# smdogroup/paropt

Measured on AMD Instinct MI355X. Metric: IP iterations/sec (KKT solve+line search), n=50M vars m=32, 1/2/4/8 GPUs, higher is better.
Workload: dtype f64

## Files before the change

paropt_amd/csrc/capi.cpp:

```cpp
#include <string.h>

#include "ip.hpp"
#include "problem.hpp"
#include "qn.hpp"

namespace po {
const char *last_error();
int ctx_create(int device, Ctx **out);
int ctx_destroy(Ctx *c);
int rccl_unique_id(void *id128);
int comm_init_rccl(Ctx *c, int rank, int size, const void *id128);
int comm_bench(Ctx *c, int count, int pure_sum, int reps, double out_us[3]);
int comm_allreduce_host(Ctx *c, double *values, int count, int op);
int rccl_version();
int comm_init_callback(Ctx *c, int rank, int size, po_allgather_fn fn, void *user);
}

using namespace po;

#define PO_CHECK_PTR(p)                         \
  do {                                          \
    if (!(p)) {                                 \
      po::set_error("null argument: %s", #p);   \
      return PO_ERR_ARG;                        \
    }                                           \
  } while (0)

static int same_layout(po_vec a, po_vec b) {
  if (a->ctx != b->ctx || a->n != b->n) {
    po::set_error("vector mismatch (different context or local size %lld vs %lld)", (long long)a->n,
                  (long long)b->n);
    return PO_ERR_ARG;
  }
  return PO_OK;
}

extern "C" {

const char *po_last_error(void) { return po::last_error(); }
const char *po_version(void) { return "paropt_amd 0.1 gfx950"; }

int po_ctx_create(int device, po_ctx *out) {
  PO_CHECK_PTR(out);
  Ctx *c = nullptr;
  int rc = ctx_create(device, &c);
  *out = static_cast<po_ctx>(c);
  return rc;
}
int po_ctx_destroy(po_ctx ctx) { return ctx_destroy(ctx); }
int po_ctx_synchronize(po_ctx ctx) {
  PO_CHECK_PTR(ctx);
  PO_HIP(hipStreamSynchronize(ctx->stream));
  return PO_OK;
}
int po_ctx_rank(po_ctx ctx, int *rank, int *size) {
  PO_CHECK_PTR(ctx);
  if (rank) *rank = ctx->rank;
  if (size) *size = ctx->size;
  return PO_OK;
}
void *po_ctx_stream(po_ctx ctx) { return ctx ? (void *)ctx->stream : nullptr; }
int po_ctx_counters(po_ctx ctx, int64_t *reductions, int64_t *launches) {
  PO_CHECK_PTR(ctx);
  if (reductions) *reductions = ctx->n_reductions;
  if (launches) *launches = ctx->n_launches;
  return PO_OK;
}
int po_ctx_sync_counters(po_ctx ctx, int64_t *flag_waits, int64_t *flag_timeouts, int64_t *allreduces,
                         int64_t *allgathers) {
  PO_CHECK_PTR(ctx);
  if (flag_waits) *flag_waits = ctx->n_flag_waits;
  if (flag_timeouts) *flag_timeouts = ctx->n_flag_timeouts;
  if (allreduces) *allreduces = ctx->n_allreduce;
  if (allgathers) *allgathers = ctx->n_allgather;
  return PO_OK;
}
int po_ctx_algorithmic_bytes(po_ctx ctx, double *total, double *user) {
  PO_CHECK_PTR(ctx);
  if (total) *total = ctx->alg_bytes;
  if (user) *user = ctx->alg_bytes_user;
  return PO_OK;
}
int po_debug_wgram_stamps(double *out8) { return po::wgram_debug_stamps(out8); }
int po_debug_set_switch(int id, int value) {
  po::dbg_switch_set(id, value);
  return PO_OK;
}

int po_ctx_set_reduction_batching(po_ctx ctx, int on) {
  PO_CHECK_PTR(ctx);
  PO_TRY(po::batch_flush(ctx));
  ctx->batch_enabled = on ? 1 : 0;
  return PO_OK;
}
int po_ctx_batched_reductions(po_ctx ctx, int64_t *batched) {
  PO_CHECK_PTR(ctx);
  if (batched) *batched = ctx->n_batched;
  return PO_OK;
}
int po_live_objects(int64_t *vectors, int64_t *bytes) {
  long v = 0;
  long long b = 0;
  po::live_objects(&v, &b);
  if (vectors) *vectors = v;
  if (bytes) *bytes = b;
  return PO_OK;
}
int po_device_count(int *count) {
  PO_CHECK_PTR(count);
  int n = 0;
  if (hipGetDeviceCount(&n) != hipSuccess) n = 0;
  *count = n;
  return PO_OK;
}
int po_options_visit_defaults(int which, po_option_visitor fn, void *user) {
  PO_CHECK_PTR(fn);
  po::Options o;
  po::Options base;
  if (which == 1) o.addTrustRegionDefaults();
  if (which == 2) o.addMMADefaults();
  if (which < 0 || which > 2) return PO_ERR_ARG;
  return o.visit(which == 0 ? nullptr : &base, fn, user);
}
int po_live_host_mirrors(int64_t *mirrors) {
  if (mirrors) *mirrors = po::live_mirrors();
  return PO_OK;
}
int po_ctx_time_mdot(po_ctx ctx, int nvecs) {
  PO_CHECK_PTR(ctx);
  ctx->time_mdot_nv = nvecs > 0 ? nvecs : 0;
  ctx->mdot_ms = 0.0;
  ctx->mdot_count = 0;
  return PO_OK;
}
int po_ctx_time_mdot_result(po_ctx ctx, double *ms_total, int64_t *launches) {
  PO_CHECK_PTR(ctx);
  if (ms_total) *ms_total = ctx->mdot_ms;
  if (launches) *launches = ctx->mdot_count;
  return PO_OK;
}
int po_ctx_time_wgram(po_ctx ctx, int on) {
  PO_CHECK_PTR(ctx);
  ctx->time_wgram = on ? 1 : 0;
  for (int i = 0; i < 2; i++) {
    ctx->wgram_ms[i] = 0.0;
    ctx->wgram_count[i] = 0;
    ctx->wgram_cols[i] = 0;
    ctx->wgram_bytes[i] = 0.0;
  }
  return PO_OK;
}
int po_ctx_time_wgram_result(po_ctx ctx, int which, double *ms_total, int64_t *launches, int *ncols,
                             double *alg_bytes_total) {
  PO_CHECK_PTR(ctx);
  if (which < 0 || which > 1) return PO_ERR_ARG;
  if (ms_total) *ms_total = ctx->wgram_ms[which];
  if (launches) *launches = ctx->wgram_count[which];
  if (ncols) *ncols = ctx->wgram_cols[which];
  if (alg_bytes_total) *alg_bytes_total = ctx->wgram_bytes[which];
  return PO_OK;
}
int po_ctx_comm_info(po_ctx ctx, int *kind, int64_t *allreduces, int64_t *allgathers) {
  PO_CHECK_PTR(ctx);
  if (kind) *kind = (int)ctx->comm_kind;
  if (allreduces) *allreduces = ctx->n_allreduce;
  if (allgathers) *allgathers = ctx->n_allgather;
// ... 1418 lines not shown
```

paropt_amd/csrc/context.cpp:

```cpp
#include <dlfcn.h>
#include <math.h>
#include <stdarg.h>
#include <execinfo.h>
#include <stdio.h>
#include <stdlib.h>
#include <string.h>
#include <time.h>

#include <algorithm>
#include <mutex>
#include <unordered_map>

#include "core.hpp"

namespace po {

static thread_local char g_err[1024] = "";
thread_local int g_last_code = 0;

void set_error(const char *fmt, ...) {
  va_list ap;
  va_start(ap, fmt);
  vsnprintf(g_err, sizeof(g_err), fmt, ap);
  va_end(ap);
  fprintf(stderr, "paropt_amd: %s\n", g_err);
}
const char *last_error() { return g_err; }

double host_now() {
  struct timespec t;
  clock_gettime(CLOCK_MONOTONIC, &t);
  return (double)t.tv_sec + 1e-9 * (double)t.tv_nsec;
}

struct SwitchDef {
  DbgSwitch id;
  const char *env;
  int dflt;
  bool presence;
};
static const SwitchDef kSwitches[] = {
    {SW_PERTURB_W, nullptr, 0, false},
    {SW_MPC_FUSE, "PAROPT_AMD_MPC_FUSE", 1, false},
    {SW_MPC_POLY, "PAROPT_AMD_MPC_POLY", 1, false},
    {SW_SPEC_DT, "PAROPT_AMD_SPEC_DT", 1, false},
    {SW_UNIFORM_BOUNDS, nullptr, 1, false},
    {SW_WGRAM_PRIO, "PAROPT_AMD_WGRAM_PRIO", 2, false},
    {SW_WGRAM_ABLATE, "PAROPT_AMD_WGRAM_ABLATE", 0, false},
    {SW_EXPLICIT_DOTS, "PAROPT_AMD_EXPLICIT_DOTS", 0, true},
    {SW_NO_RECOMPUTE, "PAROPT_AMD_NO_RECOMPUTE", 0, true},
    {SW_NO_RECOMPUTE_RHS, "PAROPT_AMD_NO_RECOMPUTE_RHS", 0, true},
    {SW_NO_FUSED_MERIT, "PAROPT_AMD_NO_FUSED_MERIT", 0, true},
    {SW_NO_LEAN_STEP, "PAROPT_AMD_NO_LEAN_STEP", 0, true},
    {SW_NO_RECOMPUTE_DT, "PAROPT_AMD_NO_RECOMPUTE_DT", 0, true},
    {SW_NO_FUSED_UPDATE, "PAROPT_AMD_NO_FUSED_UPDATE", 0, true},
    {SW_NO_CSR_GROUPS, "PAROPT_AMD_NO_CSR_GROUPS", 0, true},
    {SW_NO_FRONTS, "PAROPT_AMD_NO_FRONTS", 0, false},
    {SW_FORCE_RCCL, "PAROPT_AMD_FORCE_RCCL", 0, true},
    {SW_RCCL_ALLGATHER, "PAROPT_AMD_RCCL_ALLGATHER", 0, true},
    {SW_NO_DIRECT_RED, "PAROPT_AMD_NO_DIRECT_RED", 0, true},
    {SW_NO_FLAG_POLL, "PAROPT_AMD_NO_FLAG_POLL", 0, true},
    {SW_NO_BATCH, "PAROPT_AMD_NO_BATCH", 0, true},
    {SW_HOST_TRACE, "PAROPT_AMD_HOST_TRACE", 0, true},
    {SW_SYNC_TRACE, "PAROPT_AMD_SYNC_TRACE", 0, true},
    {SW_USER_TIMING, "PAROPT_AMD_USER_TIMING", 0, true},
    {SW_DUMP_LONG_SOLVES, "PAROPT_AMD_DUMP_LONG_SOLVES", -1, false},
};
static struct {
  int value = -1;
} g_dbg_switch[SW_COUNT];

int dbg_switch(DbgSwitch id) {
  if (g_dbg_switch[id].value >= 0) return g_dbg_switch[id].value;
  for (const SwitchDef &s : kSwitches) {
    if (s.id != id) continue;
    const char *e = s.env ? getenv(s.env) : nullptr;
    return e ? (s.presence ? 1 : atoi(e)) : s.dflt;
  }
  return 0;
}
void dbg_switch_set(int id, int value) {
  if (id >= 0 && id < SW_COUNT) g_dbg_switch[id].value = value;
}

int launch_reduce_final(Ctx *c, int nblocks, int nslots, int nsum, int nmin, int dst_off);
int launch_reduce_final_multi(Ctx *c, const Ctx::PendingRed *pend, int count);
int launch_red_publish(Ctx *c, const double *src, int count);
static int alloc_h_red(Ctx *c, size_t doubles) {
  if (c->h_red) (void)hipHostFree(c->h_red);
  c->h_red = nullptr;
  c->h_red_dev = nullptr;
  if (hipHostMalloc((void **)&c->h_red, sizeof(double) * doubles, hipHostMallocMapped | hipHostMallocCoherent) !=
      hipSuccess) {
    (void)hipGetLastError();
    c->h_red = nullptr;
    PO_HIP(hipHostMalloc((void **)&c->h_red, sizeof(double) * doubles, hipHostMallocDefault));
    c->h_red_coherent = 0;
  } else {
    c->h_red_coherent = 1;
  }
  if (dbg_switch(SW_NO_DIRECT_RED) ||
      hipHostGetDevicePointer((void **)&c->h_red_dev, c->h_red, 0) != hipSuccess) {
    (void)hipGetLastError();
    c->h_red_dev = nullptr;
  }
  if (c->h_flag && (!c->h_red_coherent || !c->h_red_dev)) {
    (void)hipHostFree(c->h_flag);
    c->h_flag = c->h_flag_dev = nullptr;
    if (c->d_ticket) (void)hipFree(c->d_ticket);
    c->d_ticket = nullptr;
  }
  if (c->h_red_dev && !c->h_flag && c->h_red_coherent && !dbg_switch(SW_NO_FLAG_POLL)) {
    if (hipHostMalloc((void **)&c->h_flag, 64, hipHostMallocMapped | hipHostMallocCoherent) == hipSuccess &&
        hipHostGetDevicePointer((void **)&c->h_flag_dev, c->h_flag, 0) == hipSuccess &&
        hipMalloc((void **)&c->d_ticket, sizeof(unsigned)) == hipSuccess &&
        hipMemset(c->d_ticket, 0, sizeof(unsigned)) == hipSuccess) {
      *c->h_flag = 0;
    } else {
      (void)hipGetLastError();
      if (c->h_flag) (void)hipHostFree(c->h_flag);
      if (c->d_ticket) (void)hipFree(c->d_ticket);
      c->h_flag = c->h_flag_dev = nullptr;
      c->d_ticket = nullptr;
    }
  }
  return PO_OK;
}


static int comm_self_test(Ctx *c);
static void free_overflow(Ctx *c, const double *keep);

struct Id128 {
  char b[PO_RCCL_ID_BYTES];
};
struct RcclApi {
  void *handle = nullptr;
  int (*GetUniqueId)(void *) = nullptr;
  int (*CommInitRank)(void **, int, Id128, int) = nullptr;
  int (*AllGather)(const void *, void *, size_t, int, void *, hipStream_t) = nullptr;
  int (*AllReduce)(const void *, void *, size_t, int, int, void *, hipStream_t) = nullptr;
  int (*CommDestroy)(void *) = nullptr;
  const char *(*GetErrorString)(int) = nullptr;
  int (*GetVersion)(int *) = nullptr;
  int version = 0;
};
static RcclApi g_rccl;

static int load_rccl() {
// ... 578 lines not shown
```

paropt_amd/csrc/core.hpp:

```cpp
#pragma once
#include <hip/hip_runtime.h>
#include <stdint.h>

#include <functional>
#include <string>
#include <vector>

#include "../../include/paropt_amd.h"

namespace po {

void set_error(const char *fmt, ...);
extern thread_local int g_last_code;

#define PO_HIP(expr)                                                                     \
  do {                                                                                   \
    hipError_t _e = (expr);                                                              \
    if (_e != hipSuccess) {                                                              \
      po::set_error("%s failed: %s (%s:%d)", #expr, hipGetErrorString(_e), __FILE__,     \
                    __LINE__);                                                           \
      return PO_ERR_HIP;                                                                 \
    }                                                                                    \
  } while (0)

#define PO_TRY(expr)            \
  do {                          \
    int _rc = (expr);           \
    if (_rc != PO_OK) return _rc; \
  } while (0)

constexpr int kBlock = 256;
constexpr int kMaxPanel = 96;
constexpr int kMaxRed = 8192;
constexpr int kWgramMaxVecs = 80;

enum CommKind { COMM_SELF = 0, COMM_RCCL = 1, COMM_CALLBACK = 2 };

struct Ctx {
  int device = 0;
  unsigned long long serial = 0;
  hipStream_t stream = nullptr;
  int num_cu = 256;
  int max_blocks = 2048;
  int rank = 0, size = 1;
  CommKind comm_kind = COMM_SELF;
  void *rccl_comm = nullptr;
  int rccl_allreduce = 1;
  long n_allreduce = 0, n_allgather = 0;
  po_allgather_fn cb_allgather = nullptr;
  void *cb_user = nullptr;
  double *d_partials = nullptr;
  double *partials_base = nullptr;
  size_t partials_cap = 0;
  size_t partials_cursor = 0;
  size_t partials_last = 0;
  double *d_red = nullptr;
  double *d_gather = nullptr;
  double *h_red = nullptr;
  double *h_red_dev = nullptr;
  unsigned long long *h_flag = nullptr, *h_flag_dev = nullptr;
  unsigned *d_ticket = nullptr;
  unsigned long long red_seq = 0, red_seq_seen = 0;
  int h_red_coherent = 0;
  long n_flag_waits = 0, n_flag_timeouts = 0;
  bool host_trace = false, host_gap_open = false;
  double host_t_sync = 0.0, host_gap_s = 0.0, host_launch_s = 0.0, host_wait_s = 0.0;
  long host_gap_n = 0, host_launch_n = 0, host_gap_n20 = 0, host_gap_long_n = 0;
  double host_gap_long_s = 0.0, host_t_launch_end = 0.0, host_inter_s = 0.0, host_inter_s30 = 0.0;
  long host_inter_n = 0, host_inter_n30 = 0;
  std::vector<double *> partials_overflow;
  hipEvent_t ev0 = nullptr, ev1 = nullptr;
  double *wide_scratch[2] = {nullptr, nullptr};
  int64_t wide_n = 0;
  hipEvent_t ev_mdot0 = nullptr, ev_mdot1 = nullptr;
  long n_reductions = 0;
  struct PendingRed {
    int off, nsum, nmin, nmax;
    double *host_out;
    const double *part;
    int nblocks;
  };
  int batch_enabled = 1;
  int batch_depth = 0;
  int batch_cursor = 0;
  std::vector<PendingRed> batch_pend;
  std::vector<std::function<void()>> batch_after;
  long n_batched = 0;
  long n_launches = 0;
  double alg_bytes = 0.0, alg_bytes_user = 0.0;
  int in_user = 0;
  int time_mdot_nv = 0;
  double mdot_ms = 0.0;
  long mdot_count = 0;
  bool mdot_timing_pending = false;
  int time_wgram = 0;
  double wgram_ms[2] = {0.0, 0.0};
  long wgram_count[2] = {0, 0};
  int wgram_cols[2] = {0, 0};
  double wgram_bytes[2] = {0.0, 0.0};
};

struct Vec {
  Ctx *ctx;
  int64_t n;
  double *d;
  int ref;
  double *h;
  int h_live = 0;
};

struct PtrTable {
  const double *p[kMaxPanel];
};
struct CoefTable {
  double a[kMaxPanel];
};
int reduce_finish(Ctx *c, int nblocks, int nsum, int nmin, int nmax, double *host_out, bool now = false,
                  double *local_out = nullptr);
bool red_direct(const Ctx *c);
int batch_flush(Ctx *c, const double *keep_partials = nullptr, size_t keep_len = 0);
void batch_abort(Ctx *c);
template <class F>
inline void after_reduce(Ctx *c, F &&f) {
  if (c->batch_depth > 0 && !c->batch_pend.empty()) {
    c->batch_after.emplace_back(std::forward<F>(f));
  } else {
    f();
  }
}
struct BatchScope {
  Ctx *c;
  bool open;
  explicit BatchScope(Ctx *c_, bool on = true) : c(c_), open(on && c_->batch_enabled) {
    if (open) c->batch_depth++;
  }
  void begin() {
    if (!open && c->batch_enabled) {
      open = true;
      c->batch_depth++;
    }
  }
  int end() {
    if (!open) return PO_OK;
    open = false;
    c->batch_depth--;
    return batch_flush(c);
  }
  int end_nested() {
    if (!open) return PO_OK;
    open = false;
    c->batch_depth--;
    return c->batch_depth > 0 ? PO_OK : batch_flush(c);
  }
  template <class F>
  int end_then(F &&post) {
    if (open) {
      open = false;
      c->batch_depth--;
      if (c->batch_depth > 0) {
        after_reduce(c, std::forward<F>(post));
        return PO_OK;
      }
      PO_TRY(batch_flush(c));
    }
    post();
    return PO_OK;
  }
  ~BatchScope() {
    if (open) {
      c->batch_depth--;
      batch_abort(c);
    }
  }
  BatchScope(const BatchScope &) = delete;
  BatchScope &operator=(const BatchScope &) = delete;
};
enum DbgSwitch {
  SW_PERTURB_W = 11, SW_MPC_FUSE = 14, SW_MPC_POLY = 15, SW_SPEC_DT = 16, SW_UNIFORM_BOUNDS = 17,
  SW_WGRAM_PRIO = 18, SW_WGRAM_ABLATE = 19, SW_EXPLICIT_DOTS = 20, SW_NO_RECOMPUTE = 21, SW_NO_RECOMPUTE_RHS = 22,
  SW_NO_FUSED_MERIT = 23, SW_NO_LEAN_STEP = 24, SW_NO_RECOMPUTE_DT = 25, SW_NO_FUSED_UPDATE = 26,
  SW_NO_CSR_GROUPS = 27, SW_NO_FRONTS = 28, SW_FORCE_RCCL = 29, SW_RCCL_ALLGATHER = 30, SW_NO_DIRECT_RED = 31,
  SW_NO_FLAG_POLL = 32, SW_NO_BATCH = 33, SW_HOST_TRACE = 34, SW_SYNC_TRACE = 35, SW_USER_TIMING = 36,
  SW_DUMP_LONG_SOLVES = 37, SW_COUNT = 38
};
int dbg_switch(DbgSwitch id);
void dbg_switch_set(int id, int value);
double host_now();
inline double host_trace_begin(Ctx *c);
inline void host_trace_end(Ctx *c, double t0);
int ensure_partials(Ctx *c, size_t doubles);
bool ctx_alive(const Ctx *c, unsigned long long serial);
inline double host_trace_begin(Ctx *c) {
  if (!c->host_trace) return 0.0;
  const double t = host_now();
  if (!c->host_gap_open && c->host_t_launch_end > 0.0) {
    const double g = t - c->host_t_launch_end;
    if (g < 500e-6) {
      c->host_inter_s += g;
      c->host_inter_n++;
      if (g > 30e-6) {
        c->host_inter_n30++;
        c->host_inter_s30 += g;
      }
    }
  }
  if (c->host_gap_open) {
    const double g = t - c->host_t_sync;
    if (g < 500e-6) {
      c->host_gap_s += g;
      c->host_gap_n++;
      if (g > 20e-6) c->host_gap_n20++;
    } else {
      c->host_gap_long_s += g;
      c->host_gap_long_n++;
    }
    c->host_gap_open = false;
  }
  return t;
}
inline void host_trace_end(Ctx *c, double t0) {
  if (!c->host_trace) return;
  c->host_t_launch_end = host_now();
  c->host_launch_s += c->host_t_launch_end - t0;
  c->host_launch_n++;
}
inline void count_bytes(Ctx *c, double streams, int64_t n) {
  const double b = 8.0 * streams * (double)n;
  c->alg_bytes += b;
  if (c->in_user) c->alg_bytes_user += b;
}
constexpr int kBpcPanel = 2;
constexpr int kBpcStream = 4;
int grid_for(Ctx *c, int64_t n);
int grid_for(Ctx *c, int64_t n, int bpc);

struct GroupCol {
  const double *w = nullptr;
  double scale = 0.0;
  unsigned period = 1, nw = 0;
  long long nwcon = 0;
};

struct GroupCols2 {
  GroupCol g[2];
  double ca[2] = {0.0, 0.0}, cb[2] = {0.0, 0.0};
  int count = 0;
};

int k_fill(Ctx *c, double *y, int64_t n, double alpha);
int k_fill_hash(Ctx *c, double *y, int64_t n, uint64_t seed, uint64_t aid, int64_t offset,
                double scale, double shift);
int k_copy(Ctx *c, double *y, const double *x, int64_t n);
int k_sign(Ctx *c, double *y, const double *x, int64_t n);
int k_scale(Ctx *c, double *y, int64_t n, double alpha);
int k_axpy(Ctx *c, double *y, double alpha, const double *x, int64_t n);
int k_panel_axpy(Ctx *c, double *y, double a, const double *x, double b, const double *alpha,
                 const double *const *V, int nv, int64_t n, const GroupCol *ybase = nullptr);
int k_panel_axpy2(Ctx *c, double *y1, double a1, const double *x1, const double *c1, double *y2, double a2,
                  const double *x2, const double *c2, const double *const *V, int nv, int64_t n);
int k_panel_lincomb(Ctx *c, double *const *dst, double a, const double *const *X, double b,
                    const double *const *Y, int nv, int64_t n);
enum Red1 { RED_DOT = 0, RED_SUMSQ = 1, RED_ASUM = 2, RED_AMAX = 3 };
int k_reduce1(Ctx *c, int kind, const double *x, const double *y, int64_t n, double *out);
int k_mdot(Ctx *c, const double *x, const double *const *V, int nv, int64_t n, double *out);
int k_minmax(Ctx *c, const double *x, int64_t n, double out[2]);
int k_stream_launch(Ctx *c, int kind, double *x, double *y, int64_t n);
int k_mdot_launch(Ctx *c, const double *x, const double *const *V, int nv, int64_t n, int *nblocks);
struct GramGroups {
  int64_t nwcon = 0, start = 0;
  int nw = 0, skip = 0;
  double alpha = 1.0;
  int ncols = 0;
  double *const *U = nullptr;
};
int k_wgram(Ctx *c, const double *d, const double *const *V, int nv, int64_t n, double *W,
            const double *const *S = nullptr, double *const *Zout = nullptr, int kpend = 0,
            double b0 = 0.0, int preweighted_last = 0, bool may_defer = false,
            const GramGroups *groups = nullptr, bool *groups_done = nullptr);
int wgram_debug_stamps(double out[8]);
int k_xgram(Ctx *c, const double *const *U, const double *const *Z, int m, int64_t w, double *out,
            bool may_defer = false);
int k_wgram_launch(Ctx *c, const double *d, const double *const *V, int nv, int64_t n,
                   int *nblocks, int *nslots, const double *const *S = nullptr,
                   double *const *Zout = nullptr, int kpend = 0, double b0 = 0.0,
                   int preweighted_last = 0, const GramGroups *groups = nullptr, bool *groups_done = nullptr);

struct Bounds {
  const double *x, *lb, *ub, *zl, *zu;
  double max_bound;
  int use_lower, use_upper;
  int lb_uni = 0, ub_uni = 0;
  double lb_c = 0.0, ub_c = 0.0;
};
inline int uniform_bound_streams(const Bounds &b) { return (b.lb_uni ? 1 : 0) + (b.ub_uni ? 1 : 0); }
struct ResidualSums {
  double comp_prod = 0, comp_count = 0, l1_rx = 0, l1_rzl = 0, l1_rzu = 0, l2_rx = 0, l2_rzl = 0, l2_rzu = 0;
  double max_rx = 0, max_rzl = 0, max_rzu = 0;
  double spec_max_rzl = 0, spec_max_rzu = 0;
  double *as_array() { return &comp_prod; }
};
static_assert(sizeof(ResidualSums) == 13 * sizeof(double), "k_kkt_res writes 13 slots");
struct KktResArgs {
  Bounds b;
  const double *g = nullptr;
  const double *const *A = nullptr;
  const double *z = nullptr;
  int nc = 0;
  double beta_mu = 0.0;
  int64_t n = 0;
  double *rx = nullptr;
  double *out = nullptr;
  double *yqn = nullptr;
  double beta_mu2 = -1.0;
  const GroupCol *gcol = nullptr;
  double gcoef = 0.0;
  struct Update {
    double *zl = nullptr;
    const double *pzl = nullptr;
    double *zu = nullptr;
    const double *pzu = nullptr;
    double a = 0.0, eps = 0.0;
    const double *va = nullptr;
    double az = 0.0;
    double *acz = nullptr;
    double az_acz = 0.0;
    const double *pxs = nullptr, *xold = nullptr;
    double beta_mu_step = 0.0;
    double *dinv_out = nullptr, *t_out = nullptr;
    double spec_diag = 0.0, spec_beta_mu = 0.0;
  } update;
};
int k_kkt_res(Ctx *c, const KktResArgs &o);
int k_kkt_res_update(Ctx *c, const KktResArgs &o);
int k_res_norms(Ctx *c, const Bounds &b, double beta_mu, int64_t n, double out[11]);
int k_dinv(Ctx *c, const Bounds &b, double diag, int64_t n, double *dinv,
           const double *hdiag = nullptr);
int k_d1s(Ctx *c, const Bounds &b, const double *bx, const double *dinv, double alpha, double beta_mu,
          int64_t n, double *t);
int k_solve2s(Ctx *c, const Bounds &b, const double *t, const double *dinv, const double *coef,
              const double *const *P, int nv, double alpha, double beta_mu, int full, double tau, int64_t n,
              double *px, double *pzl, double *pzu, double out[2]);
int k_d1(Ctx *c, const Bounds &b, const double *rx, const double *dinv, double beta_mu, int64_t n,
         double *t, const double *cl = nullptr, const double *cu = nullptr);
int k_dinv_d1(Ctx *c, const Bounds &b, double diag, const double *hdiag, const double *rx, double beta_mu,
              int64_t n, double *dinv, double *t, int raw = 0);
int k_corrector(Ctx *c, const Bounds &b, const double *px, const double *pzl, const double *pzu,
                int64_t n, double *cl, double *cu);
constexpr int kCorrDotsMax = 15;
int k_corr_d1_dots(Ctx *c, const Bounds &b, const double *px, const double *pzl, const double *pzu, const double *rx,
                   const double *dinv, double beta_mu, const double *const *V, int nv, int64_t n, double *t,
                   double *out);
struct CorrectorSums {
  double S10 = 0, S01 = 0, S11 = 0, ppos = 0, pneg = 0, gpx = 0, pxpx = 0, pos_log = 0, neg_log = 0;
  double max_x = 0, max_z = 0;
  double px_amax = 0;
  double *as_array() { return &S10; }
};
static_assert(sizeof(CorrectorSums) == 12 * sizeof(double), "k_solve2c writes 12 slots");
struct Solve2cArgs {
  Bounds b;
  const double *t = nullptr, *dinv = nullptr;
  const double *alpha = nullptr;
  const double *const *P = nullptr;
  int nv = 0;
  double beta_mu = 0.0, tau = 0.0;
  int64_t n = 0;
  double *px = nullptr, *pzl = nullptr, *pzu = nullptr;
  double *va = nullptr;
  int nca = 0;
  const double *g = nullptr;
  int want_logs = 0;
  double *out = nullptr;
};
int k_solve2c(Ctx *c, const Solve2cArgs &o);
struct Solve2Args {
  Bounds b;
  const double *t = nullptr, *dinv = nullptr;
// ... 131 lines not shown
```

paropt_amd/csrc/ip.cpp:

```cpp
#include "ip.hpp"

#include <math.h>
#include <stdio.h>
#include <stdlib.h>
#include <string.h>

#include <algorithm>
#include <chrono>

namespace po {

static const int LS_SUCCESS = 1, LS_FAILURE = 2, LS_MIN_STEP = 4, LS_MAX_ITERS = 8,
                 LS_NO_IMPROVEMENT = 16, LS_SHORT_STEP = 32;

InteriorPoint::InteriorPoint(Problem *p)
    : prob(p), ctx(p->ctx), n(p->nlocal), c(p->ncon), qn(nullptr), x(nullptr), zl(nullptr),
      zu(nullptr), lb(nullptr), ub(nullptr), g(nullptr), fobj(0.0), barrier_param(0.1),
      rho_penalty_search(0.0), niter(0), neval(0), ngeval(0),
      iter_cb(nullptr),
      iter_cb_user(nullptr), px(nullptr), pzl(nullptr), pzu(nullptr), Dinv(nullptr), rx(nullptr),
      tvec(nullptr), xt(nullptr), y_qn(nullptr), s_qn(nullptr), vA(nullptr), qn_created(false), qn_owned(true),
      comp_prod(0), comp_count(0), max_rx(0), max_rzl(0), max_rzu(0),
      corrector_active(false), norm_type(0), phase_t0(0) {
  qn_handle.qn = nullptr;
// ... 506 lines not shown
      mi = std::max(mi, fabs(r.z[i]));
      md = std::max(md, std::max(fabs(r.zs[i]), fabs(r.zt[i])));
    }
    if (use_lower) md = std::max(md, max_rzl);
    if (use_upper) md = std::max(md, max_rzu);
    if (has_w) {
      mi = std::max(mi, w_maxs[0]);
      md = std::max(md, std::max(std::max(w_maxs[1], w_maxs[2]), std::max(w_maxs[3], w_maxs[4])));
    }
  } else if (norm_type == 1) {
    mp = l1_rx;
    for (int i = 0; i < c; i++) {
      mp += fabs(r.s[i]);
      mp += fabs(r.t[i]);
      mi += fabs(r.z[i]);
      md += fabs(r.zs[i]);
      md += fabs(r.zt[i]);
    }
    if (use_lower) md += l1_rzl;
    if (use_upper) md += l1_rzu;
    if (has_w) {
      mi += w_sums[1];
      md += w_sums[3] + w_sums[4] + w_sums[5] + w_sums[6];
    }
  } else {
    double prime = 0.0, infeas = 0.0, dual = 0.0;
    for (int i = 0; i < c; i++) {
      prime += r.s[i] * r.s[i] + r.t[i] * r.t[i];
      infeas += r.z[i] * r.z[i];
      dual += r.zs[i] * r.zs[i] + r.zt[i] * r.zt[i];
    }
    mp = l2_rx + prime;
    mi = infeas;
    md = dual;
    if (use_lower) md += l2_rzl;
    if (use_upper) md += l2_rzu;
    if (has_w) {
      mi += w_sums[2];
      md += w_sums[3] * w_sums[3] + w_sums[4] * w_sums[4] + w_sums[5] * w_sums[5] +
            w_sums[6] * w_sums[6];
    }
    mp = sqrt(mp);
    mi = sqrt(mi);
    md = sqrt(md);
  }
  *max_prime = mp;
  *max_dual = md;
  *max_infeas = mi;
  *res_norm = std::max(mp, std::max(md, mi));
}

double InteriorPoint::compFromSums(double prod, double count, const Dense &v,
                                   double wprod) const {
  prod = prod / options.real("rel_bound_barrier");
  if (has_w) {
    prod += wprod;
    count += 2.0 * nw_global;
  }
  for (int i = 0; i < c; i++) {
    prod += v.s[i] * v.zs[i] + v.t[i] * v.zt[i];
    count += 2.0;
  }
  return count != 0.0 ? prod / count : 0.0;
}

int InteriorPoint::getComplementarity(double *comp) {
  double out[11];
  PO_TRY(k_res_norms(ctx, bounds(), 0.0, n, out));
  double wprod = 0.0;
  if (has_w) PO_TRY(wCompStep(0.0, 0.0, &wprod));
  *comp = compFromSums(out[0], out[1], vars, wprod);
  return PO_OK;
}

int InteriorPoint::formDinvAndRhs(double diag, bool use_hdiag, const double *rhs_mu, int kz, RhsFormed *formed) {
  const double *h = use_hdiag ? hdiag->d : nullptr;
  const double bmu = rhs_mu ? options.real("rel_bound_barrier") * (*rhs_mu) : 0.0;
  const bool want_t = rhs_mu && !has_w && c + kz > 0;
  const bool want_raw_d1 = has_w && rhs_mu && !corrector_active;
  const bool have_spec_dt = scratch_flags.spec_dt_valid;
  scratch_flags.spec_dt_valid = false;
  scratch_flags.t_is_plain_dinv_d1 = false;
  *formed = RHS_NONE;
  if (want_t) {
    const bool left_behind = have_spec_dt && !use_hdiag && spec_dt_diag == diag && spec_dt_bmu == bmu;
    if (!left_behind) PO_TRY(k_dinv_d1(ctx, bounds(), diag, h, rx->d, bmu, n, Dinv->d, tvec->d));
    scratch_flags.t_is_plain_dinv_d1 = !use_hdiag;
    t0_diag = diag;
    *formed = RHS_T;
  } else if (want_raw_d1) {
    PO_TRY(k_dinv_d1(ctx, bounds(), diag, h, rx->d, bmu, n, Dinv->d, d1v->d, 1));
    *formed = RHS_RAW_D1;
  } else {
    PO_TRY(k_dinv(ctx, bounds(), diag, n, Dinv->d, h));
  }
  return PO_OK;
}

int InteriorPoint::gramPass(const GramPlan &plan, bool *groups_done) {
  const int m = (int)plan.V.size(), mt = m + (plan.with_t ? 1 : 0), k = plan.kform;
  const bool with_t = plan.with_t;
  std::vector<const double *> V(plan.V);
  if (with_t) V.push_back(tvec->d);
  Wt_buf.assign((size_t)mt * mt, 0.0);
  PO_TRY(k_wgram(ctx, Dinv->d, V.data(), mt, n, Wt_buf.data(), k > 0 ? plan.S.data() : nullptr,
                 k > 0 ? plan.Zout.data() : nullptr, k, plan.b0, with_t ? 1 : 0, plan.may_defer, plan.groups,
                 groups_done));
  t0dots.assign(with_t ? m : 0, 0.0);
  after_reduce(ctx, [this, m, mt, k, with_t] {
    auto at = [&](int i) { return k == 0 ? i : (i < c ? k + i : i - c); };
    for (int j = 0; j < m; j++)
      for (int i = 0; i < m; i++) kkt.W[i + (size_t)m * j] = Wt_buf[at(i) + (size_t)mt * at(j)];
    for (int i = 0; with_t && i < m; i++) t0dots[i] = Wt_buf[at(i) + (size_t)mt * m];
  });
  return PO_OK;
}

int InteriorPoint::setUpKKTSystem(bool use_qn, bool diag_only, const double *rhs_mu) {
  if (qn) PO_TRY(refreshQuasiNewton());
  step_flags.ptpx_valid = false;
  scratch_flags.t0_valid = false;
  const bool use_hdiag = options.integer("use_diag_hessian") && hdiag;
  const double b0 = (!use_hdiag && qn && (use_qn || diag_only)) ? qn->diag() : 0.0;
  const bool with_z = use_qn && !diag_only;
  RhsFormed rhs = RHS_NONE;
  PO_TRY(formDinvAndRhs(b0 + options.real("qn_sigma"), use_hdiag, rhs_mu, (qn && with_z) ? qn->size() : 0, &rhs));
  const bool fuse_t = rhs == RHS_T, raw_d1_w = rhs == RHS_RAW_D1;
  GramPlan plan;
  std::vector<const double *> Yp, Sp;
  std::vector<double *> Zo;
  double b0z = 0.0;
  const bool fuse_z = qn && with_z && !has_w && qn->pendingZ(&Yp, &Sp, &Zo, &b0z) && !Yp.empty() && Yp.size() <= 12 &&
                      c + (int)Yp.size() + (fuse_t ? 1 : 0) <= kWgramMaxVecs;
  int k = 0;
  std::vector<const double *> P;
  if (fuse_z) {
    plan.kform = k = (int)Yp.size();
    plan.V = Yp;
    for (Vec *a : Ac) plan.V.push_back(a->d);
    plan.S = Sp;
    plan.Zout = Zo;
    plan.b0 = b0z;
  } else {
    plan.V = P = panel(with_z, &k);
  }
  const int m = c + k;
  kkt.k = k;
  bool fuse_tw = false;
  BatchScope wbatch(ctx, has_w && prob->reductionsBatchable());
  if (has_w) {
    PO_TRY(prob->sparseFactorFromSlacks(x, Dinv, wv(), Cw));
    fuse_tw = rhs_mu && m > 0 && m + 1 <= kWgramMaxVecs && !corrector_active;
    if (fuse_tw) {
      PO_TRY(computeResidualW(*rhs_mu, true, true));
      if (!raw_d1_w)
        PO_TRY(k_d1(ctx, bounds(), rx->d, nullptr, options.real("rel_bound_barrier") * (*rhs_mu), n, d1v->d));
      PO_TRY(applyK0(d1v->d, wd2->d, tvec, wyw));
    }
  }
  GramGroups gram_groups;
  std::vector<double *> Ugs;
  if (has_w && m > 0 && prob->sparseGramGroups(x, &gram_groups)) {
    PO_TRY(panelImageVectors(m, Ugs));
    gram_groups.ncols = m;
    gram_groups.U = Ugs.data();
    plan.groups = &gram_groups;
  }
  plan.with_t = (fuse_t || fuse_tw) && m > 0 && m + 1 <= kWgramMaxVecs;
  plan.may_defer = wbatch.open;
  bool panel_done = false;
  kkt.W.assign((size_t)m * m, 0.0);
  t0dots.clear();
  if (m > 0) PO_TRY(gramPass(plan, &panel_done));
  if (fuse_z) qn->pendingZDone();
  if (plan.with_t) {
    scratch_flags.t0_valid = true;
    t0_mu = *rhs_mu;
  }
  if (has_w) PO_TRY(sparseGramCorrection(P, m, fuse_tw ? d1v : tvec, wbatch.open, panel_done));
  PO_TRY(wbatch.end());
  if (m > 1 && debug_keep_schur && dbg_switch(SW_PERTURB_W) != 0) {
    kkt.W[1] *= 1.0 + 1e-9;
    kkt.W[m] = kkt.W[1];
  }
  const double *d0 = nullptr, *M = nullptr;
  if (k > 0) {
    double b0_;
    qn->getCompactMat(&b0_, &d0, &M, nullptr);
  }
  kkt.factor(vars, d0, M, debug_keep_schur ? &Gmat0 : nullptr, debug_keep_schur ? &Ce0 : nullptr);
  if (k == 0) Ce0.clear();
  return PO_OK;
}

int InteriorPoint::solveKKT(const Dense &b, double mu, bool use_qn, bool refine_pass, double tau,
                            Dense &out, bool fuse_residual) {
  const double beta_mu = options.real("rel_bound_barrier") * mu;
  const int k = (qn && use_qn) ? qn->size() : 0;
  PO_TRY(kkt.checkWidth(k));
  const int m = c + k;
  std::vector<const double *> P;
  bool have_panel = false;
  auto need_panel = [&]() {
    if (!have_panel) {
      int k2 = 0;
      P = panel(use_qn, &k2);
      have_panel = true;
    }
  };
  const bool corr = corrector_active && !refine_pass;
  const bool corr_fused = corr && corrector_fused && m >= 1 && m <= kCorrDotsMax;
  const double *cl = (corr && !corr_fused) ? s_qn->d : nullptr;
  const double *cu = (corr && !corr_fused) ? y_qn->d : nullptr;
  if (corr && corrector_fused && !corr_fused) {
    set_error("internal: fused corrector solve with a panel of %d columns", m);
    return PO_ERR_ARG;
  }
  const bool have_t0 = !refine_pass && scratch_flags.t0_valid && t0_mu == mu && !corr && (int)t0dots.size() == m;
  std::vector<double> dots(m > 0 ? m : 1, 0.0);
  if (corr_fused) {
    need_panel();
    PO_TRY(k_corr_d1_dots(ctx, bounds(), px->d, pzl->d, pzu->d, rx->d, Dinv->d, beta_mu, P.data(), m, n, tvec->d,
                          dots.data()));
  } else {
    if (!refine_pass && !have_t0) PO_TRY(k_d1(ctx, bounds(), rx->d, Dinv->d, beta_mu, n, tvec->d, cl, cu));
    if (have_t0) {
      for (int i = 0; i < m; i++) dots[i] = t0dots[i];
    } else if (refine_pass && step_flags.tdots_valid && (int)tdots.size() == m) {
      dots = tdots;
    } else if (m > 0) {
      need_panel();
      PO_TRY(k_mdot(ctx, tvec->d, P.data(), m, n, dots.data()));
    }
  }
  if (!refine_pass) scratch_flags.first_t_recomputable = have_t0 && scratch_flags.t_is_plain_dinv_d1;
  if (!refine_pass) scratch_flags.t0_valid = false;
  const bool deferred = refine_pass && step_flags.step_deferred;
  const Bordered::Sol sol = solveBordered(b, dots.data(), refine_pass);
  const bool seq_lin = options.integer("sequential_linear_method");
  const int kq = (qn && !seq_lin) ? qn->size() : 0;
  const bool fuse = fuse_residual && !refine_pass && forms.analytic_panel_dots && kq == k &&
                    !options.integer("use_diag_hessian") && !inexact_newton_step && m <= kMaxPanel;
  step_flags.vA_valid = true;
  std::vector<double> coef(m > 0 ? m : 1, 0.0);
  double diag = options.real("qn_sigma");
  if (fuse) PO_TRY(residualCoefs(qn && !seq_lin ? RES_QN : RES_SIGMA, sol.coef.data(), ptpx.data() + c, k, coef, &diag));
  need_panel();
  const SolvePass sp{P, sol.coef, m, beta_mu, tau};
  if (fuse && m > 0 && !corr) {
    PO_TRY(fusedFirstPass(sp, coef, diag));
  } else if (deferred) {
    PO_TRY(recomputingRefinementPass(sp, corr));
  } else if (corr_fused) {
    PO_TRY(correctorSolve(sp));
  } else {
    PO_TRY(storedStepSolve(sp, refine_pass, fuse ? coef.data() : nullptr, diag, cl, cu));
  }
  step_flags.residual_fused = fuse;
  kkt.backSubstitute(1.0, b, vars, sol, true, out);
  return PO_OK;
}

Bordered::Sol InteriorPoint::solveBordered(const Dense &b, const double *dots, bool refine_pass) {
  stepWillChange();
  Bordered::Sol sol;
  kkt.solve(1.0, b, vars, dots, &sol);
  kkt.panelDots(dots, sol, refine_pass, &ptpx);
  step_flags.ptpx_valid = true;
  return sol;
}

int InteriorPoint::fusedFirstPass(const SolvePass &sp, const std::vector<double> &coef, double diag) {
  const int m = sp.m;
  std::vector<double> out(m + 2, 0.0);
  const bool defer = forms.recompute_first_step;
  double *tp_out = !defer ? tvec->d : (forms.recompute_rhs ? nullptr : xt->d);
  const bool redo_dt1 = forms.recompute_dt && defer && forms.recompute_rhs && scratch_flags.first_t_recomputable;
  PO_TRY(k_solve2_dots(ctx, {.b = bounds(), .t = redo_dt1 ? nullptr : tvec->d, .dinv = Dinv->d,
                             .alpha = sp.alpha.data(), .coef2 = coef.data(), .P = sp.P.data(), .nv = m,
                             .beta_mu = sp.beta_mu, .tau = sp.tau, .rx = rx->d, .diag = diag, .n = n, .px = px->d,
                             .pzl = pzl->d, .pzu = pzu->d, .tout = tp_out, .va = vA->d, .nca = c, .out = out.data(),
                             .store_step = defer ? 0 : 1, .dinv_diag = t0_diag}));
  tdots.assign(out.begin(), out.begin() + m);
  step_flags.tdots_valid = true;
  step_mins[0] = out[m];
  step_mins[1] = out[m + 1];
  step_flags.step_deferred = defer;
  if (defer) {
    alpha_first = sp.alpha;
    coef_first = coef;
    diag_first = diag;
  }
  return PO_OK;
}

int InteriorPoint::recomputingRefinementPass(const SolvePass &sp, bool corr) {
  const bool take_merit = forms.fuse_merit && forms.recompute_rhs && !corr;
  const bool lean = forms.lean_step && lean_step_allowed && take_merit && iterate_flags.iterate_logs_valid;
  const bool redo_dt = forms.recompute_dt && forms.recompute_rhs && scratch_flags.first_t_recomputable;
  if (lean) {
    step_flags.pz_stored = false;
    step_beta_mu = sp.beta_mu;
  }
  PO_TRY(k_solve2r(ctx, {.b = bounds(), .t1 = redo_dt ? nullptr : tvec->d,
                         .t2 = forms.recompute_rhs ? nullptr : xt->d, .dinv = Dinv->d, .a1 = alpha_first.data(),
                         .a2 = sp.alpha.data(), .P = sp.P.data(), .nv = sp.m, .beta_mu = sp.beta_mu, .tau = sp.tau,
                         .n = n, .px = px->d, .pzl = lean ? nullptr : pzl->d, .pzu = lean ? nullptr : pzu->d,
                         .va = vA->d, .nca = c, .out = step_mins, .ar = coef_first.data(), .rx = rx->d,
                         .diag = diag_first, .g = take_merit ? g->d : nullptr,
                         .merit_out = take_merit ? fused_merit.as_array() : nullptr, .dinv_diag = t0_diag}));
  if (take_merit) {
    after_reduce(ctx, [this] {
      step_mins[0] = fused_merit.max_x;
      step_mins[1] = fused_merit.max_z;
      step_flags.fused_merit_valid = true;
    });
  }
  return PO_OK;
}

int InteriorPoint::correctorSolve(const SolvePass &sp) {
  const bool want_logs = !iterate_flags.iterate_logs_valid;
  PO_TRY(k_solve2c(ctx, {.b = bounds(), .t = tvec->d, .dinv = Dinv->d, .alpha = sp.alpha.data(), .P = sp.P.data(),
                         .nv = sp.m, .beta_mu = sp.beta_mu, .tau = sp.tau, .n = n, .px = px->d, .pzl = pzl->d,
                         .pzu = pzu->d, .va = vA->d, .nca = c, .g = g->d, .want_logs = want_logs ? 1 : 0,
                         .out = corr_out.as_array()}));
  after_reduce(ctx, [this, want_logs] {
    const CorrectorSums &o = corr_out;
    fused_merit = {.S10 = o.S10, .S01 = o.S01, .S11 = o.S11, .ppos = o.ppos, .pneg = o.pneg, .gpx = o.gpx,
                   .pxpx = o.pxpx, .max_x = o.max_x, .max_z = o.max_z, .px_amax = o.px_amax};
    step_mins[0] = o.max_x;
    step_mins[1] = o.max_z;
    if (want_logs) {
      iterate_logs[0] = o.pos_log;
      iterate_logs[1] = o.neg_log;
      iterate_flags.iterate_logs_valid = true;
    }
    step_flags.fused_merit_valid = true;
  });
  return PO_OK;
}

int InteriorPoint::storedStepSolve(const SolvePass &sp, bool refine_pass, const double *coef2, double diag,
                                   const double *cl, const double *cu) {
  return k_solve2(ctx, {.b = bounds(), .t = tvec->d, .dinv = Dinv->d, .alpha = sp.alpha.data(), .P = sp.P.data(),
                        .nv = sp.m, .beta_mu = sp.beta_mu, .refine = refine_pass ? 1 : 0, .tau = sp.tau, .n = n,
                        .px = px->d, .pzl = pzl->d, .pzu = pzu->d, .out = step_mins, .coef2 = coef2, .rx = rx->d,
                        .diag = diag, .tout = tvec->d, .va = vA->d, .nca = c, .cl = cl, .cu = cu});
}

int InteriorPoint::computeKKTStepWithRefinement(double mu, bool use_qn, double tau) {
  const int nref = options.integer("iterative_refinement_steps");
  const double beta_mu = options.real("rel_bound_barrier") * mu;
  const bool with_qn = qn && !options.integer("sequential_linear_method");
  const int mq = c + (with_qn ? qn->size() : 0);
  const bool diag_hess = options.integer("use_diag_hessian") && (!has_w || hdiag);
  const ResTerm term = (!has_w && inexact_newton_step) ? RES_HVEC
                       : diag_hess                     ? RES_HDIAG
                       : with_qn                       ? RES_QN
                                                       : RES_SIGMA;
  if (has_w && !(scratch_flags.t0_valid && t0_mu == mu)) PO_TRY(computeResidualW(mu));
  denseResidual(mu, res);
  PO_TRY(has_w ? solveKKTW(res, mu, use_qn, false, tau, step, nref > 0)
               : solveKKT(res, mu, use_qn, false, tau, step, nref > 0));
  for (int it = 0; it < nref; it++) {
    LazyPanel Pq{this, with_qn};
    if (has_w) Pq.get();
    std::vector<double> dots;
    PO_TRY(stepPanelDots(Pq, dots));
    std::vector<double> coef(mq + 2, 0.0);
    double diag = 0.0;
    PO_TRY(residualCoefs(term, step.z.data(), dots.data() + c, mq - c, coef, &diag));
    int mres = mq;
    if (term == RES_HVEC || term == RES_HDIAG) {
      Pq.get().push_back(xt->d);
      mres++;
    }
    if (!(it == 0 && step_flags.residual_fused)) {
      if (has_w) {
        if (prob->setSparseJacobianTranspose(1.0, x, wstepv[0], tvec) != 0) return PO_ERR_USER;
        Pq.get().push_back(tvec->d);
        coef[mres++] = 1.0;
      }
      PO_TRY(k_res_step(ctx, bounds(), rx->d, px->d, pzl->d, pzu->d, has_w ? nullptr : Dinv->d, coef.data(),
                        Pq.get().data(), mres, diag, beta_mu, n, has_w ? d1v->d : tvec->d));
    }
    if (has_w) {
      PO_TRY(computeResidualW(mu, false));
      if (prob->addSparseJacobian(-1.0, x, px, wresv[0]) != 0) return PO_ERR_USER;
      PO_TRY(k_w_res_step(ctx, wv(), wp(), wr(), nw, wd2->d));
      scratch_flags.wd2_ready = true;
    }
    Dense r2;
    r2.resize(c);
    denseResidual(mu, r2);
    denseResStep(vars, step, dots.data(), r2);
    PO_TRY(has_w ? solveKKTW(r2, mu, use_qn, true, tau, refine) : solveKKT(r2, mu, use_qn, true, tau, refine));
    for (int i = 0; i < c; i++) {
      step.z[i] += refine.z[i];
      step.s[i] += refine.s[i];
      step.t[i] += refine.t[i];
      step.zs[i] += refine.zs[i];
      step.zt[i] += refine.zt[i];
    }
  }
  sx = sz = 1.0;
  return PO_OK;
}

int InteriorPoint::checkKKTStep(int iteration, double mu) {
  const double beta_mu = options.real("rel_bound_barrier") * mu;
  if (!step_flags.pz_stored) {
    PO_TRY(k_form_pz(ctx, bounds(), px->d, step_beta_mu, n, pzl->d, pzu->d));
    step_flags.pz_stored = true;
  }
  const bool seq_lin = options.integer("sequential_linear_method");
  int kq = 0;
  std::vector<const double *> Pq = panel(qn && !seq_lin, &kq);
  const int mq = c + kq;
  std::vector<double> dots(mq > 0 ? mq : 1, 0.0), coef(mq > 0 ? mq : 1, 0.0);
  if (mq > 0) PO_TRY(k_mdot(ctx, px->d, Pq.data(), mq, n, dots.data()));
  double diag = 0.0;
  const bool with_qn = qn && !seq_lin && !options.integer("use_diag_hessian");
  PO_TRY(residualCoefs(with_qn ? RES_QN : RES_SIGMA, step.z.data(), dots.data() + c, kq, coef, &diag));
  if (has_w) {
    if (prob->setSparseJacobianTranspose(1.0, x, wstepv[0], xt) != 0) return PO_ERR_USER;
    Pq.push_back(xt->d);
    coef.push_back(1.0);
  }
  double mx[3];
  PO_TRY(computeResidual(mu, true));
  PO_TRY(k_step_check(ctx, bounds(), rx->d, px->d, pzl->d, pzu->d, coef.data(), Pq.data(), (int)Pq.size(), diag,
                      beta_mu, n, mx));
  Dense r;
  r.resize(c);
  denseResidual(mu, r);
  denseResStep(vars, step, dots.data(), r);
  double mz = 0.0, ms = 0.0, mt = 0.0, mzs = 0.0, mzt = 0.0;
  for (int i = 0; i < c; i++) {
    mz = std::max(mz, fabs(r.z[i]));
    ms = std::max(ms, fabs(r.s[i]));
    mt = std::max(mt, fabs(r.t[i]));
    mzs = std::max(mzs, fabs(r.zs[i]));
    mzt = std::max(mzt, fabs(r.zt[i]));
  }
  if (ctx->rank == 0) {
    char line[640];
    snprintf(line, sizeof(line),
             "\nResidual step check for iteration %d:\n"
             "max |stationarity (x block)|:             %10.4e\n"
             "max |dense constraints (z block)|:        %10.4e\n"
             "max |slack duals (s block)|:              %10.4e\n"
             "max |slack duals (t block)|:              %10.4e\n"
             "max |slack complementarity (zs block)|:   %10.4e\n"
             "max |slack complementarity (zt block)|:   %10.4e\n"
             "max |lower-bound complementarity (zl)|:   %10.4e\n"
             "max |upper-bound complementarity (zu)|:   %10.4e\n",
             iteration, mx[0], mz, ms, mt, mzs, mzt, mx[1], mx[2]);
    history += line;
  }
  return PO_OK;
}

int InteriorPoint::checkGradients(double dh, std::string *report) {
  scratchLent();
  return prob->checkGradients(dh, x, options.integer("use_hvec_product"), xt, tvec, report);
// ... 1342 lines not shown
```

paropt_amd/csrc/ip.hpp:

```cpp
#pragma once
#include <stdlib.h>
#include <map>
#include <string>
#include <vector>

#include "bordered.hpp"
#include "problem.hpp"
#include "qn.hpp"

namespace po {

class Options {
 public:
  enum Type { STR = 1, BOOL = 2, INT = 3, FLOAT = 4, ENUM = 5 };
  struct Entry {
    Type type;
    std::string s;
    int i = 0, ilo = 0, ihi = 0;
    double f = 0, flo = 0, fhi = 0;
    std::vector<std::string> choices;
  };
  Options();
  void addTrustRegionDefaults();
  void addMMADefaults();
  int set(const char *name, const char *value);
  int set(const char *name, int value);
  int set(const char *name, double value);
  const char *str(const char *name) const;
  int integer(const char *name) const;
  double real(const char *name) const;
  bool has(const char *name) const { return e.count(name) > 0; }
  int visit(const Options *skip, po_option_visitor fn, void *user) const;
  void adoptExtras(const Options &src, const Options &base);

 private:
  std::map<std::string, Entry> e;
};

class InteriorPoint {
 public:
  InteriorPoint(Problem *prob);
  ~InteriorPoint();
  int allocate();
  const std::vector<int> &gPivots() const { return kkt.gpiv; }
  Vec *lowerBounds() { return lb; }
  Vec *upperBounds() { return ub; }
  void clearUniformBounds() { bounds_uni[0] = bounds_uni[1] = 0; }
  int checkFlag() const { return check_flag; }
  int clampCounts(double out[8]);
  int checkKKTStep(int iteration, double mu);

  Options options;
  int optimize(const char *checkpoint);
  void getOptimizedPoint(Vec **x, const double **z, Vec **zl, Vec **zu);
  void getOptimizedSlacks(const double **s, const double **t, const double **zs, const double **zt);
  void getOptimizedSparse(Vec *v[5]);
  void getIterationCounters(int *niter_, int *neval_, int *ngeval_);
  double getBarrierParameter() const { return barrier_param; }
  int getComplementarity(double *comp);
  void setPenaltyGamma(double gamma);
  void setPenaltyGammaArray(const double *gamma);
  int resetDesignAndBounds();
  void resetQuasiNewtonHessian();
  int setQuasiNewton(CompactQuasiNewton *qn_);
  int resetProblemInstance(Problem *p);
  int writeSolutionFile(const char *filename);
  int readSolutionFile(const char *filename);
  int debugKKTStep(double mu);
  int debugSetState(const double *z, const double *s, const double *t, const double *zs, const double *zt, double mu);
  int debugKKT(double mu, int mode, double tau);
  std::vector<double> Gmat0, Ce0;
  bool debug_keep_schur = false;
  double debug_norms[4] = {0, 0, 0, 0};
  const std::vector<double> &gramMatrix() const { return kkt.W; }
  const std::vector<int> &cPivots() const { return kkt.cpiv; }
  const double *stepMins() const { return step_mins; }
  Vec *dinvVec() { return Dinv; }
  Vec *rxVec() { return rx; }
  void flushHistory();
  int checkGradients(double dh, std::string *report);
  int checkMeritFuncGradient(Vec *xpt, double dh, double out[2]);
  int setHvecFiniteDifference(int mode, int central, double rel_step);
  void getHvecFiniteDifferenceCount(int *products, int *evaluations) const;
  double hvecFiniteDifferenceStep() const { return hvec_fd_h; }
  int evalHvec(const double *z, Vec *zw, Vec *p, Vec *hvec);

  Problem *prob;
  Ctx *ctx;
  int64_t n;
  int c;
  CompactQuasiNewton *qn;
  po_qn_s qn_handle;

  Vec *x, *zl, *zu, *lb, *ub, *g;
  std::vector<Vec *> Ac;
  Dense vars, res, step, refine;
  double fobj, barrier_param, rho_penalty_search;
  std::vector<double> cvals;
  int niter, neval, ngeval, nhvec;

  po_ip_iteration_fn iter_cb;
  void *iter_cb_user;
  std::string history;
  std::vector<std::string> phase_names;
  std::vector<double> phase_seconds;
  std::string phase_names_joined;
  bool user_timing = dbg_switch(SW_USER_TIMING) != 0;

  Vec *px, *pzl, *pzu;

  int64_t nw;
  bool has_w;
  double nw_global;
  Vec *wvar[5], *wresv[5], *wstepv[5];

 private:
  Vec *Dinv, *rx, *tvec, *xt, *y_qn, *s_qn;
  Vec *vA;
  std::vector<double> gamma_s, gamma_t;
  int use_lower, use_upper;
  bool qn_created;
  bool qn_owned;

  Bordered kkt;
  std::vector<double> Wt_buf, W2_buf;
  Bordered::Sol solveBordered(const Dense &b, const double *dots, bool refine_pass);
  struct SolvePass {
    const std::vector<const double *> &P;
    const std::vector<double> &alpha;
    int m;
    double beta_mu, tau;
  };

  struct StepFlags {
    bool ptpx_valid = false;
    bool tdots_valid = false;
    bool merit_cache_valid = false;
    bool fused_merit_valid = false;
    bool px_amax_valid = false;
    bool w_comp_valid = false;
    bool w_merit_cache_valid = false;
    bool vA_valid = false;
    bool residual_fused = false;
    bool pz_stored = true;
    bool step_deferred = false;
    bool px_first_only = false;
  } step_flags;
  std::vector<double> ptpx;
  std::vector<double> tdots;
  MeritSums merit_cache;
  FusedMeritSums fused_merit;
  CorrectorSums corr_out;
  double px_amax_w = 0.0;
  double w_step_out[5] = {0, 0, 0, 0, 0}, w_comp_poly[3] = {0, 0, 0}, w_merit_cache[10] = {0};
  bool lean_step_allowed = false;
  double step_beta_mu = 0.0;
  std::vector<double> alpha_first, coef_first;
  double diag_first = 0.0;
  double step_mins[2];
  double sx = 1.0, sz = 1.0;

  struct ScratchFlags {
    bool spec_dt_valid = false;
    bool t0_valid = false;
    bool t_is_plain_dinv_d1 = false;
    bool first_t_recomputable = false;
    bool wd2_ready = false;
    bool panel_valid = false;
  } scratch_flags;
  bool spec_dt_want = false;
  double spec_dt_diag = 0.0, spec_dt_bmu = 0.0, spec_dt_mu = 0.0;
  double t0_mu = 0.0;
  std::vector<double> t0dots;
  double t0_diag = 0.0;

  struct IterateFlags {
    bool ac_valid = false;
    bool acz_valid = false;
    bool cwx_valid = false;
    bool trial_cw_valid = false;
    bool iterate_logs_valid = false;
    bool trial_logs_valid = false;
    bool residual_cached = false;
    bool spec_valid = false;
    bool s_qn_from_trial = false;
  } iterate_flags;
  static const int kAczRefresh = 16;
  Vec *acz = nullptr;
  int acz_age = 0;
  double trial_logs[2] = {0, 0}, iterate_logs[2] = {0, 0};
  bool spec_enabled = false;
  double spec_mu = 0.0, spec_max[2] = {0.0, 0.0};
  double s_qn_a = 0.0;

  void stepWillChange() { step_flags = {}; }
  void scratchLent() { scratch_flags = {}; }
  void iterateReplaced() { iterate_flags = {}; }
  void stateReplaced() {
    stepWillChange();
    scratchLent();
    iterateReplaced();
  }

  ResidualSums res_out;
  double wres_out[12] = {0};
  double comp_prod, comp_count, max_rx, max_rzl, max_rzu;
  double l1_rx = 0, l1_rzl = 0, l1_rzu = 0, l2_rx = 0, l2_rzl = 0, l2_rzu = 0;
  bool corrector_active;
  bool corrector_fused = false;
  int norm_type;

  Vec *hdiag;
  std::vector<Vec *> gmresW;
  bool inexact_newton_step;
  int gatherCounts(int64_t mine, std::vector<int64_t> *all);
  int solutionFileOffsets(int64_t *nvars_total, int64_t *var_off, int64_t *nw_total, int64_t *w_off);
  int ensureHdiag();
  int solveKKTAlpha(const double *bx, double alpha, const Dense &b, double mu, bool use_qn, bool full,
                    double tau, Dense &out);
  int evalObjBarrierDeriv(const Dense &p, double *pmerit);
  int solveKKTAlphaW(const double *bx, double alpha, const Dense &b, double mu, bool use_qn, bool full,
                     double tau, Dense &out);
  Vec *wscalev[5];
  double w_merit_last[10];
  int computeKKTGMRESStep(double rtol, double atol, bool use_qn, double tau, int *gmres_iters);

  int hvec_mode = PO_HVEC_EXACT, hvec_central = 0;
  double hvec_rel = 0.0;
  bool hvec_fd_active = false;
  int hvec_fd_products = 0, hvec_fd_evals = 0;
  double hvec_fd_h = 0.0;
  Vec *hvec_xp = nullptr;
  std::vector<Vec *> hvec_work[2];
  Vec *hvec_csr_data = nullptr, *hvec_csr_cw = nullptr;
  int64_t hvec_csr_nnz = 0;
  int hvecProduct(const double *z, Vec *zw, Vec *p, Vec *hvec);
  int hvecFiniteDifference(const double *z, Vec *zw, Vec *p, Vec *hvec);
  int hvecScratch(int sides, int nc);
  int hvecEvalAt(double a, Vec *p, int side, bool with_jac);

  Vec *gsw, *gtw, *Cw, *wd2, *wyw, *wtmp, *wtmp2;
  Vec *cwx = nullptr;
  int sparseConAtIterate(const double **cw);
  Vec *d1v;
  std::vector<Vec *> Uw;
  GramForm panel_form = {false, false};
  std::vector<Vec *> Yw;
  std::vector<const double *> correctionPanel(int m) const;
  double w_sums[7], w_maxs[5];
  double nextMonotoneMu() const;
  WVars wv() const;
  WVars wr() const;
  WVars wp() const;
  int allocateW();
  int applyK0(const double *bx, const double *bw, Vec *yx, Vec *yw);
  int computeResidualW(double mu, bool norms = true, bool with_d2 = false);
  int sparseGramCorrection(const std::vector<const double *> &P, int m, Vec *work = nullptr, bool may_defer = false,
                           bool panel_done = false);
  int panelImageVectors(int m, std::vector<double *> &U);
  int solveKKTW(const Dense &b, double mu, bool use_qn, bool refine_pass, double tau, Dense &out,
                bool fuse_residual = false);
  int fusedFirstPassW(const SolvePass &sp, int k, double mins_x[2], double mins_w[2]);
  int correctionPanelSolve(const SolvePass &sp, bool refine_pass, bool first_px_only, const double *cl,
                           const double *cu, double mins_x[2], double mins_w[2]);
  int blockSolveFallback(const SolvePass &sp, bool refine_pass, const double *cl, const double *cu, double mins_x[2],
                         double mins_w[2]);
  int initLeastSquaresMultipliersW();
  int wCompStep(double ax, double az, double *prod);

  Bounds bounds() const;
  std::vector<const double *> panel(bool use_qn, int *k) const;
  struct LazyPanel {
    const InteriorPoint *ip;
    bool use_qn;
    bool asked = false;
    std::vector<const double *> P;
    std::vector<const double *> &get();
  };
  int stepPanelDots(LazyPanel &P, std::vector<double> &dots);
  std::vector<double> compactInverse(const double *ztp, int kq) const;
  enum ResTerm { RES_SIGMA, RES_QN, RES_HVEC, RES_HDIAG };
  int residualCoefs(ResTerm term, const double *z, const double *ztpx, int kq, std::vector<double> &coef,
                    double *diag);

  int createQuasiNewton();
  int refreshQuasiNewton();
  int initAndCheckDesignAndBounds();
  int initLeastSquaresMultipliers();
  int initAffineStepMultipliers();
  void denseResidual(double mu, Dense &r) const;
  struct MultUpdate {
    double a = 0.0, az = 0.0, eps = 0.0;
    bool acz_follow = false;
  };
  int computeResidual(double mu, bool vectors, Vec *yqn_complete = nullptr, const MultUpdate *upd = nullptr);
  void resNorms(const Dense &r, double *max_prime, double *max_dual, double *max_infeas,
                double *res_norm) const;
  double compFromSums(double prod, double count, const Dense &v, double wprod = 0.0) const;
  int setUpKKTSystem(bool use_qn, bool diag_only = false, const double *rhs_mu = nullptr);
  enum RhsFormed { RHS_NONE, RHS_T, RHS_RAW_D1 };
  int formDinvAndRhs(double diag, bool use_hdiag, const double *rhs_mu, int kz, RhsFormed *formed);
  struct GramPlan {
    std::vector<const double *> V;
    int kform = 0;
    std::vector<const double *> S;
    std::vector<double *> Zout;
    double b0 = 0.0;
    bool with_t = false;
    const GramGroups *groups = nullptr;
    bool may_defer = false;
  };
  int gramPass(const GramPlan &plan, bool *groups_done);
  int solveKKT(const Dense &b, double mu, bool use_qn, bool refine_pass, double tau, Dense &out,
               bool fuse_residual = false);
  int fusedFirstPass(const SolvePass &sp, const std::vector<double> &coef, double diag);
  int recomputingRefinementPass(const SolvePass &sp, bool corr);
  int correctorSolve(const SolvePass &sp);
  int storedStepSolve(const SolvePass &sp, bool refine_pass, const double *coef2, double diag, const double *cl,
                      const double *cu);
  int computeKKTStepWithRefinement(double mu, bool use_qn, double tau);
  int mehrotraStep(bool use_qn, double comp, bool corrector, double min_frac, double abs_res_tol, double *tau_out);
  int scaleKKTStep(double tau, double comp, double *alpha_x, double *alpha_z, int *ceq,
                   bool inexact = false);
  int evalMeritInitDeriv(double max_x, double *merit, double *pmerit);
  double evalMeritFromSums(double fk, const double *ck, const double *sk, const double *tk,
                           double pos, double neg, const double *wsums = nullptr) const;
  int lineSearch(double alpha_min, double *alpha, double m0, double dm0, int *fail);
  int computeStepAndUpdate(double alpha, int eval_obj_con, int perform_qn_update, int *update_type);
  void phaseBegin();
  void phaseEnd(const char *name);
  double phase_t0;
  static const int kUserRing = 16;
  hipEvent_t user_ev[2 * kUserRing];
  int user_pending = 0;
  bool user_events_ready = false;
  double user_seconds = 0.0;
  void userBegin();
  void userEnd();
  void userHarvest();
  struct Forms {
    bool analytic_panel_dots;
    bool fuse_merit;
    bool lean_step;
    bool recompute_dt;
    bool recompute_first_step;
    bool recompute_rhs;
    bool fuse_mult_update;
  };
  static Forms readForms();
  const Forms forms = readForms();
  int check_flag = 0;
  int bounds_uni[2] = {0, 0};
  double bounds_val[2] = {0.0, 0.0};
};

}

struct po_ip_s {
  po::InteriorPoint *ip;
};
```

paropt_amd/csrc/ip_gmres.cpp:

```cpp
#include <math.h>

#include <algorithm>

#include "ip.hpp"

namespace po {

int InteriorPoint::ensureHdiag() {
  if (hdiag) return PO_OK;
  hdiag = vec_new(ctx, n);
  return hdiag ? PO_OK : PO_ERR_HIP;
}

int InteriorPoint::solveKKTAlpha(const double *bx, double alpha, const Dense &b, double mu, bool use_qn,
                                 bool full, double tau, Dense &out) {
  const double beta_mu = options.real("rel_bound_barrier") * mu;
  int k = 0;
  std::vector<const double *> P = panel(use_qn, &k);
  PO_TRY(kkt.checkWidth(k));
  const int m = c + k;
  PO_TRY(k_d1s(ctx, bounds(), bx, Dinv->d, alpha, beta_mu, n, tvec->d));
  std::vector<double> dots(m > 0 ? m : 1, 0.0);
  if (m > 0) PO_TRY(k_mdot(ctx, tvec->d, P.data(), m, n, dots.data()));
  Bordered::Sol sol;
  kkt.solve(alpha, b, vars, dots.data(), &sol);
  const std::vector<double> &coef = sol.coef;
  stepWillChange();
  kkt.panelDots(dots.data(), sol, false, &ptpx);
  step_flags.ptpx_valid = true;
  PO_TRY(k_solve2s(ctx, bounds(), tvec->d, Dinv->d, coef.data(), P.data(), m, alpha, beta_mu, full ? 1 : 0, tau,
                   n, px->d, pzl->d, pzu->d, step_mins));
  kkt.backSubstitute(alpha, b, vars, sol, full, out);
  return PO_OK;
}

int InteriorPoint::solveKKTAlphaW(const double *bx, double alpha, const Dense &b, double mu, bool use_qn,
                                  bool full, double tau, Dense &out) {
  const double beta_mu = options.real("rel_bound_barrier") * mu;
  int k = 0;
  std::vector<const double *> P = panel(use_qn, &k);
  PO_TRY(kkt.checkWidth(k));
  const int m = c + k;
  WVars ws{wscalev[0]->d, wscalev[1]->d, wscalev[2]->d, wscalev[3]->d, wscalev[4]->d};
  PO_TRY(k_d1s(ctx, bounds(), bx, nullptr, alpha, beta_mu, n, d1v->d));
  PO_TRY(k_w_scale5(ctx, ws, wr(), alpha, nw));
  PO_TRY(k_w_d2(ctx, wv(), ws, nw, wd2->d));
  PO_TRY(applyK0(d1v->d, wd2->d, tvec, wyw));
  std::vector<double> dots(m > 0 ? m : 1, 0.0);
  if (m > 0) PO_TRY(k_mdot(ctx, tvec->d, P.data(), m, n, dots.data()));
  Bordered::Sol sol;
  kkt.solve(alpha, b, vars, dots.data(), &sol);
  const std::vector<double> &coef = sol.coef;
  stepWillChange();
  kkt.panelDots(dots.data(), sol, false, &ptpx);
  step_flags.ptpx_valid = true;
  double mins_w[2] = {1.0, 1.0};
  if (!full && k > 0) {
    if (c > 0) {
      PO_TRY(k_panel_axpy(ctx, xt->d, 1.0, d1v->d, 0.0, sol.yz.data(), P.data(), c, n));
      PO_TRY(applyK0(xt->d, wd2->d, tvec, wyw));
    }
    PO_TRY(k_w_step(ctx, wv(), ws, wyw->d, 0, tau, wp(), nw, mins_w));
    PO_TRY(k_panel_axpy(ctx, d1v->d, 0.0, nullptr, 1.0, coef.data(), P.data(), m, n));
    PO_TRY(applyK0(d1v->d, wd2->d, tvec, wtmp2));
  } else {
    if (m > 0) PO_TRY(k_panel_axpy(ctx, d1v->d, 0.0, nullptr, 1.0, coef.data(), P.data(), m, n));
    PO_TRY(applyK0(d1v->d, wd2->d, tvec, wyw));
    PO_TRY(k_w_step(ctx, wv(), ws, wyw->d, 0, tau, wp(), nw, mins_w));
  }
  double mins_x[2] = {1.0, 1.0};
  PO_TRY(k_solve2s(ctx, bounds(), tvec->d, Dinv->d, coef.data(), P.data(), 0, alpha, beta_mu, full ? 1 : 0, tau,
                   n, px->d, pzl->d, pzu->d, mins_x));
  step_mins[0] = std::min(mins_x[0], mins_w[0]);
  step_mins[1] = std::min(mins_x[1], mins_w[1]);
  kkt.backSubstitute(alpha, b, vars, sol, full, out);
  return PO_OK;
}

int InteriorPoint::evalObjBarrierDeriv(const Dense &p, double *pmerit_) {
  const double beta = options.real("rel_bound_barrier");
  double out[6];
  PO_TRY(k_merit0(ctx, bounds(), px->d, 1.0, g->d, n, out));
  double ppos = out[2] * beta, pneg = out[3] * beta;
  if (has_w) {
    const double *cw = nullptr;
    PO_TRY(sparseConAtIterate(&cw));
    PO_TRY(k_fill(ctx, wtmp2->d, nw, 0.0));
    if (prob->addSparseJacobian(1.0, x, px, wtmp2) != 0) return PO_ERR_USER;
    PO_TRY(k_w_merit(ctx, wv(), wp(), 1.0, gsw->d, gtw->d, cw, wtmp2->d, nw, w_merit_last));
    ppos += w_merit_last[2];
    pneg += w_merit_last[3];
  }
  for (int i = 0; i < c; i++) {
    if (p.s[i] > 0.0) ppos += p.s[i] / vars.s[i]; else pneg += p.s[i] / vars.s[i];
    if (p.t[i] > 0.0) ppos += p.t[i] / vars.t[i]; else pneg += p.t[i] / vars.t[i];
  }
  double pmerit = out[4] - barrier_param * (ppos + pneg);
  for (int i = 0; i < c; i++) pmerit += gamma_s[i] * p.s[i] + gamma_t[i] * p.t[i];
  if (has_w) pmerit += w_merit_last[6] + w_merit_last[7];
  *pmerit_ = pmerit;
  return PO_OK;
}

// ... 172 lines not shown
```

paropt_amd/csrc/kernels.hip:

```cpp
#include "core.hpp"

#include <math.h>
#include <stdlib.h>
#include <string.h>

namespace po {

#define PO_PAIR_LOOP(q, n)                                                                 \
  const int64_t _npairs = ((n) + 1) >> 1;                                                  \
  for (int64_t q = (int64_t)blockIdx.x * blockDim.x + threadIdx.x; q < _npairs;            \
       q += (int64_t)gridDim.x * blockDim.x)

typedef double f64x2l __attribute__((ext_vector_type(2)));
__device__ __forceinline__ double2 ld2(const double *__restrict__ p, int64_t q, int64_t n) {
#ifndef PO_LD2_PLAIN
  const f64x2l v = __builtin_nontemporal_load(reinterpret_cast<const f64x2l *>(p + 2 * q));
  return make_double2(v.x, v.y);
#else
  return *reinterpret_cast<const double2 *>(p + 2 * q);
#endif
}
#ifndef PO_ST2_PLAIN
#define PO_ST2_NT 1
#endif
typedef double f64x2s __attribute__((ext_vector_type(2)));
__device__ __forceinline__ void st2(double *__restrict__ p, int64_t q, int64_t n, double2 v) {
  if (2 * q + 1 >= n) v.y = 0.0;
#ifdef PO_ST2_NT
  __builtin_nontemporal_store((f64x2s){v.x, v.y}, reinterpret_cast<f64x2s *>(p + 2 * q));
#else
  *reinterpret_cast<double2 *>(p + 2 * q) = v;
#endif
}

typedef double f64x4 __attribute__((ext_vector_type(4)));
typedef double f64x2 __attribute__((ext_vector_type(2)));

__device__ __forceinline__ f64x2 ld_stream(const double *p) {
  return __builtin_nontemporal_load(reinterpret_cast<const f64x2 *>(p));
}

enum { OP_SUM = 0, OP_MIN = 1, OP_MAX = 2 };

template <int OP>
__device__ __forceinline__ double combine(double a, double b) {
  if (OP == OP_SUM) return a + b;
  if (OP == OP_MIN) return fmin(a, b);
  return fmax(a, b);
}

template <int OP>
__device__ __forceinline__ double wave_reduce(double v) {
#pragma unroll
  for (int o = 32; o > 0; o >>= 1) v = combine<OP>(v, __shfl_xor(v, o, 64));
  return v;
}

template <int N, int OP>
__device__ __forceinline__ void block_reduce_store(double (&a)[N], double *__restrict__ partials,
                                                   int slot0, double *sm) {
  const int lane = threadIdx.x & 63, wave = threadIdx.x >> 6;
#pragma unroll
  for (int j = 0; j < N; j++) {
    double v = wave_reduce<OP>(a[j]);
    if (lane == 0) sm[wave * N + j] = v;
  }
  __syncthreads();
  if (threadIdx.x < N) {
    const int j = threadIdx.x;
    double v = combine<OP>(combine<OP>(sm[j], sm[N + j]), combine<OP>(sm[2 * N + j], sm[3 * N + j]));
    partials[(size_t)(slot0 + j) * gridDim.x + blockIdx.x] = v;
  }
  __syncthreads();
}

__device__ __forceinline__ void red_raise_flag(volatile unsigned long long *flag, unsigned long long seq,
                                               unsigned *ticket) {
  if (!flag) return;
  __threadfence_system();
  __syncthreads();
  if (threadIdx.x == 0) {
    const unsigned t = atomicAdd(ticket, 1u);
    if (t == gridDim.x - 1) {
// ... 623 lines not shown
  __shared__ double sm[4 * NVB];
  double acc[NVB];
  const double *vp[NVB];
#pragma unroll
  for (int j = 0; j < NVB; j++) {
    acc[j] = 0.0;
    vp[j] = V.p[j0 + j];
  }
  PO_PAIR_LOOP(q, n) {
    const f64x2 xv = *reinterpret_cast<const f64x2 *>(x + 2 * q);
#pragma unroll
    for (int j = 0; j < NVB; j++) {
      const f64x2 w = ld_stream(vp[j] + 2 * q);
      acc[j] = fma(xv.x, w.x, fma(xv.y, w.y, acc[j]));
    }
  }
  block_reduce_store<NVB, OP_SUM>(acc, partials, j0, sm);
}

#define PO_MDOT_CASE(NVB)                                                          \
  case NVB:                                                                        \
    PO_LAUNCH(mdot_kernel<NVB>, grid, x, pt, j0, n, c->d_partials);                \
    break;

int k_mdot_launch(Ctx *c, const double *x, const double *const *V, int nv, int64_t n, int *nblocks) {
  count_bytes(c, nv + 1, n);
  if (nv > kMaxPanel) {
    set_error("mdot of %d vectors exceeds kMaxPanel=%d", nv, kMaxPanel);
    return PO_ERR_ARG;
  }
  const int grid = grid_for(c, n, 5);
  PO_TRY(ensure_partials(c, (size_t)grid * (nv + 32)));
  PtrTable pt;
  CoefTable ct;
  fill_tables(nullptr, V, nv, &ct, &pt);
  int j0 = 0;
  while (j0 < nv) {
    const int rem = nv - j0;
    const int w = rem >= 32 ? 32 : (rem >= 24 ? 24 : (rem >= 16 ? 16 : rem));
    switch (w) {
      PO_MDOT_CASE(1) PO_MDOT_CASE(2) PO_MDOT_CASE(3) PO_MDOT_CASE(4) PO_MDOT_CASE(5)
      PO_MDOT_CASE(6) PO_MDOT_CASE(7) PO_MDOT_CASE(8) PO_MDOT_CASE(9) PO_MDOT_CASE(10)
      PO_MDOT_CASE(11) PO_MDOT_CASE(12) PO_MDOT_CASE(13) PO_MDOT_CASE(14) PO_MDOT_CASE(15)
      PO_MDOT_CASE(16) PO_MDOT_CASE(24) PO_MDOT_CASE(32)
    }
    j0 += w;
  }
  *nblocks = grid;
  return PO_OK;
}

int k_mdot(Ctx *c, const double *x, const double *const *V, int nv, int64_t n, double *out) {
  if (nv <= 0) return PO_OK;
  if (nv > kMaxPanel) {
    for (int j0 = 0; j0 < nv; j0 += kMaxPanel)
      PO_TRY(k_mdot(c, x, V + j0, nv - j0 > kMaxPanel ? kMaxPanel : nv - j0, n, out + j0));
    return PO_OK;
  }
  int grid = 0;
  const bool timed = c->time_mdot_nv == nv;
  if (timed && c->mdot_timing_pending) PO_TRY(batch_flush(c));
  if (timed) PO_HIP(hipEventRecord(c->ev_mdot0, c->stream));
  PO_TRY(k_mdot_launch(c, x, V, nv, n, &grid));
  if (timed) PO_HIP(hipEventRecord(c->ev_mdot1, c->stream));
  const bool defer = timed && c->batch_depth > 0;
  PO_TRY(reduce_finish(c, grid, nv, 0, 0, out, timed && !defer));
  if (timed) {
    auto harvest = [c] {
      float ms = 0.0f;
      if (hipEventSynchronize(c->ev_mdot1) == hipSuccess &&
          hipEventElapsedTime(&ms, c->ev_mdot0, c->ev_mdot1) == hipSuccess) {
        c->mdot_ms += ms;
        c->mdot_count++;
      }
      c->mdot_timing_pending = false;
    };
    if (defer) c->mdot_timing_pending = true;
    after_reduce(c, harvest);
  }
  return PO_OK;
}


struct BE {
  bool L, U;
  double xl, xu, zl, zu;
};
__device__ __forceinline__ BE bound_elem(double x, double lb, double ub, double zl, double zu,
                                         double maxb, int use_lower, int use_upper) {
  BE e;
  e.L = use_lower && (lb > -maxb);
  e.U = use_upper && (ub < maxb);
  e.xl = e.L ? (x - lb) : 1.0;
  e.xu = e.U ? (ub - x) : 1.0;
  e.zl = zl;
  e.zu = zu;
  return e;
}
#define PO_MAKE_BOUNDS(b, q, n)                                                          \
  const bool _has2 = (2 * q + 1 < n);                                                    \
  const BE e0 = bound_elem(_x.x, _lb.x, _ub.x, _zl.x, _zu.x, (b).max_bound, (b).use_lower, \
                           (b).use_upper);                                               \
  BE e1 = bound_elem(_x.y, _lb.y, _ub.y, _zl.y, _zu.y, (b).max_bound, (b).use_lower,     \
                     (b).use_upper);                                                     \
  if (!_has2) {                                                                          \
    e1.L = false;                                                                        \
    e1.U = false;                                                                        \
    e1.xl = 1.0;                                                                         \
    e1.xu = 1.0;                                                                         \
  }
__device__ __forceinline__ double2 ld2_bound(const double *__restrict__ p, int uni, double v, int64_t q, int64_t n) {
  return uni ? make_double2(v, v) : ld2(p, q, n);
}
#define PO_LD2_LB(b, q, n) ld2_bound((b).lb, (b).lb_uni, (b).lb_c, q, n)
#define PO_LD2_UB(b, q, n) ld2_bound((b).ub, (b).ub_uni, (b).ub_c, q, n)
#define PO_LOAD_BOUNDS(b, q, n)                                                         \
  const double2 _x = ld2((b).x, q, n), _lb = PO_LD2_LB(b, q, n), _ub = PO_LD2_UB(b, q, n), \
                _zl = ld2((b).zl, q, n), _zu = ld2((b).zu, q, n);                        \
  PO_MAKE_BOUNDS(b, q, n)

__device__ __forceinline__ void res_bound_acc(const BE &e, double beta_mu, double *sums, double *maxs,
                                              int il1, int il2, int imax) {
  if (e.L) {
    sums[0] += e.zl * e.xl;
    sums[1] += 1.0;
    const double r = fabs(-(e.xl * e.zl - beta_mu));
    sums[il1] += r;
    sums[il2] += r * r;
    maxs[imax] = fmax(maxs[imax], r);
  }
  if (e.U) {
    sums[0] += e.zu * e.xu;
    sums[1] += 1.0;
    const double r = fabs(-(e.xu * e.zu - beta_mu));
    sums[il1 + 1] += r;
    sums[il2 + 1] += r * r;
    maxs[imax + 1] = fmax(maxs[imax + 1], r);
  }
}
__device__ __forceinline__ void res_bound_max2(const BE &e, double beta_mu2, double *m2) {
  if (e.L) m2[0] = fmax(m2[0], fabs(-(e.xl * e.zl - beta_mu2)));
  if (e.U) m2[1] = fmax(m2[1], fabs(-(e.xu * e.zu - beta_mu2)));
}
__global__ void __launch_bounds__(kBlock)
    kkt_res_kernel(Bounds b, const double *__restrict__ g, PtrTable A, CoefTable z, int nc,
                   double beta_mu, int64_t n, double *__restrict__ rx, double *__restrict__ yqn,
                   double beta_mu2, GroupCol gcol, double gcoef, double *__restrict__ partials) {
  __shared__ double sm[4 * 8];
  double sums[8] = {0.0, 0.0, 0.0, 0.0, 0.0, 0.0, 0.0, 0.0};
  double maxs[5] = {0.0, 0.0, 0.0, 0.0, 0.0};
  PO_PAIR_LOOP(q, n) {
    PO_LOAD_BOUNDS(b, q, n);
    const double2 gv = ld2(g, q, n);
    double2 yv = make_double2(0.0, 0.0);
    if (yqn) yv = ld2(yqn, q, n);
    double2 r;
    r.x = (b.use_lower ? _zl.x : 0.0);
    r.y = (b.use_lower ? _zl.y : 0.0);
    if (b.use_upper) {
      r.x += -1.0 * _zu.x;
      r.y += -1.0 * _zu.y;
    }
    r.x += -1.0 * gv.x;
    r.y += -1.0 * gv.y;
    GRaw graw;
    if (gcol.w) graw = gcol_request(gcol, q, n);
    double2 ps = panel_sum(A, z, nc, q);
    if (gcol.w) {
      const f64x2 gcv = gcol_value(gcol, graw);
      ps.x += gcoef * gcv.x;
      ps.y += gcoef * gcv.y;
    }
    r.x += ps.x;
    r.y += ps.y;
    if (!_has2) r.y = 0.0;
    st2(rx, q, n, r);
    if (yqn) {
      const double cl = b.use_lower ? 1.0 : 0.0, cu = b.use_upper ? -1.0 : 0.0;
      yv.x = __dadd_rn(yv.x, __fma_rn(-1.0, r.x, __fma_rn(cu, _zu.x, __fma_rn(cl, _zl.x, 0.0))));
      yv.y = __dadd_rn(yv.y, __fma_rn(-1.0, r.y, __fma_rn(cu, _zu.y, __fma_rn(cl, _zl.y, 0.0))));
      st2(yqn, q, n, yv);
    }
    maxs[0] = fmax(maxs[0], fmax(fabs(r.x), fabs(r.y)));
    sums[2] += fabs(r.x) + fabs(r.y);
    sums[5] += r.x * r.x + r.y * r.y;
    res_bound_acc(e0, beta_mu, sums, maxs, 3, 6, 1);
    res_bound_acc(e1, beta_mu, sums, maxs, 3, 6, 1);
    if (beta_mu2 >= 0.0) {
      res_bound_max2(e0, beta_mu2, maxs + 3);
      res_bound_max2(e1, beta_mu2, maxs + 3);
    }
  }
  block_reduce_store<8, OP_SUM>(sums, partials, 0, sm);
  if (beta_mu2 >= 0.0) {
    block_reduce_store<5, OP_MAX>(maxs, partials, 8, sm);
  } else {
    double m3[3] = {maxs[0], maxs[1], maxs[2]};
    block_reduce_store<3, OP_MAX>(m3, partials, 8, sm);
  }
}

int k_kkt_res(Ctx *c, const KktResArgs &o) {
  PO_TRY(gcol_check(o.gcol, o.n, "k_kkt_res"));
  if (o.nc > kMaxPanel) {
    const double *w = nullptr, one = 1.0;
    PO_TRY(collapse_range(c, 0, o.z, o.A, 0, o.nc, o.n, &w));
    KktResArgs o1 = o;
    o1.A = &w;
    o1.z = &one;
    o1.nc = 1;
    return k_kkt_res(c, o1);
  }
  count_bytes(c, 7 + o.nc + (o.yqn ? 2 : 0) - uniform_bound_streams(o.b), o.n);
  const int grid = grid_for(c, o.n, kBpcPanel);
  PO_TRY(ensure_partials(c, (size_t)grid * 13));
  PtrTable pt;
  CoefTable ct;
  fill_tables(o.z, o.A, o.nc, &ct, &pt);
  if (o.gcol) count_bytes(c, 1.0, o.gcol->nwcon);
  PO_LAUNCH(kkt_res_kernel, grid, o.b, o.g, pt, ct, o.nc, o.beta_mu, o.n, o.rx, o.yqn, o.beta_mu2,
            o.gcol ? *o.gcol : GroupCol(), o.gcoef, c->d_partials);
  return reduce_finish(c, grid, 8, 0, o.beta_mu2 >= 0.0 ? 5 : 3, o.out);
}

__global__ void __launch_bounds__(kBlock)
    res_norms_kernel(Bounds b, double beta_mu, int64_t n, double *__restrict__ partials) {
  __shared__ double sm[4 * 8];
  double sums[8] = {0.0, 0.0, 0.0, 0.0, 0.0, 0.0, 0.0, 0.0};
  double maxs[3] = {0.0, 0.0, 0.0};
  PO_PAIR_LOOP(q, n) {
    PO_LOAD_BOUNDS(b, q, n);
    res_bound_acc(e0, beta_mu, sums, maxs, 3, 6, 1);
    res_bound_acc(e1, beta_mu, sums, maxs, 3, 6, 1);
  }
  block_reduce_store<8, OP_SUM>(sums, partials, 0, sm);
  block_reduce_store<3, OP_MAX>(maxs, partials, 8, sm);
}

int k_res_norms(Ctx *c, const Bounds &b, double beta_mu, int64_t n, double out[11]) {
  count_bytes(c, 5 - uniform_bound_streams(b), n);
  const int grid = grid_for(c, n);
  PO_TRY(ensure_partials(c, (size_t)grid * 11));
  PO_LAUNCH(res_norms_kernel, grid, b, beta_mu, n, c->d_partials);
  return reduce_finish(c, grid, 8, 0, 3, out);
}

__device__ __forceinline__ double dinv_elem(const BE &e, double diag) {
  double v = diag;
  if (e.L) v += e.zl / e.xl;
  if (e.U) v += e.zu / e.xu;
  return 1.0 / v;
}
__global__ void __launch_bounds__(kBlock)
    dinv_kernel(Bounds b, double diag, const double *__restrict__ hdiag, int64_t n,
                double *__restrict__ dinv) {
  PO_PAIR_LOOP(q, n) {
    PO_LOAD_BOUNDS(b, q, n);
    double2 h = make_double2(0.0, 0.0);
    if (hdiag) h = ld2(hdiag, q, n);
    st2(dinv, q, n, make_double2(dinv_elem(e0, diag + h.x), dinv_elem(e1, diag + h.y)));
  }
}
int k_dinv(Ctx *c, const Bounds &b, double diag, int64_t n, double *dinv, const double *hdiag) {
  count_bytes(c, 6 + (hdiag ? 1 : 0) - uniform_bound_streams(b), n);
  if (n <= 0) return PO_OK;
  PO_LAUNCH(dinv_kernel, grid_for(c, n), b, diag, hdiag, n, dinv);
  return PO_OK;
}

__device__ __forceinline__ double d1_elem(const BE &e, double rx, double beta_mu, double cl = 0.0,
                                          double cu = 0.0) {
  double d1 = rx;
  if (e.L) d1 += (-(e.xl * e.zl - beta_mu) - cl) / e.xl;
  if (e.U) d1 -= (-(e.xu * e.zu - beta_mu) + cu) / e.xu;
  return d1;
}
__global__ void __launch_bounds__(kBlock)
    d1_kernel(Bounds b, const double *__restrict__ rx, const double *__restrict__ dinv,
              double beta_mu, const double *__restrict__ cl, const double *__restrict__ cu, int64_t n,
              double *__restrict__ t) {
  PO_PAIR_LOOP(q, n) {
    PO_LOAD_BOUNDS(b, q, n);
    const double2 r = ld2(rx, q, n);
    const double2 dv = dinv ? ld2(dinv, q, n) : make_double2(1.0, 1.0);
    double2 c0 = make_double2(0.0, 0.0), c1 = c0;
    if (cl) {
      c0 = ld2(cl, q, n);
      c1 = ld2(cu, q, n);
    }
    st2(t, q, n,
        make_double2(dv.x * d1_elem(e0, r.x, beta_mu, c0.x, c1.x),
                     dv.y * d1_elem(e1, r.y, beta_mu, c0.y, c1.y)));
  }
}
int k_d1(Ctx *c, const Bounds &b, const double *rx, const double *dinv, double beta_mu, int64_t n,
         double *t, const double *cl, const double *cu) {
  count_bytes(c, 7 + (dinv ? 1 : 0) + (cl ? 2 : 0) - uniform_bound_streams(b), n);
  if (n <= 0) return PO_OK;
  PO_LAUNCH(d1_kernel, grid_for(c, n), b, rx, dinv, beta_mu, cl, cu, n, t);
  return PO_OK;
}

__global__ void __launch_bounds__(kBlock)
    dinv_d1_kernel(Bounds b, double diag, const double *__restrict__ hdiag, const double *__restrict__ rx,
                   double beta_mu, int64_t n, double *__restrict__ dinv, double *__restrict__ t, int raw) {
  PO_PAIR_LOOP(q, n) {
    PO_LOAD_BOUNDS(b, q, n);
    double2 h = make_double2(0.0, 0.0);
    if (hdiag) h = ld2(hdiag, q, n);
    const double2 r = ld2(rx, q, n);
    const double2 dv = make_double2(dinv_elem(e0, diag + h.x), dinv_elem(e1, diag + h.y));
    st2(dinv, q, n, dv);
    const double w0 = raw ? 1.0 : dv.x, w1 = raw ? 1.0 : dv.y;
    st2(t, q, n, make_double2(w0 * d1_elem(e0, r.x, beta_mu), w1 * d1_elem(e1, r.y, beta_mu)));
  }
}
int k_dinv_d1(Ctx *c, const Bounds &b, double diag, const double *hdiag, const double *rx, double beta_mu,
              int64_t n, double *dinv, double *t, int raw) {
  count_bytes(c, 8 + (hdiag ? 1 : 0) - uniform_bound_streams(b), n);
  if (n <= 0) return PO_OK;
  PO_LAUNCH(dinv_d1_kernel, grid_for(c, n), b, diag, hdiag, rx, beta_mu, n, dinv, t, raw);
  return PO_OK;
}

__global__ void __launch_bounds__(kBlock)
    corrector_kernel(Bounds b, const double *__restrict__ px, const double *__restrict__ pzl,
                     const double *__restrict__ pzu, int64_t n, double *__restrict__ cl,
                     double *__restrict__ cu) {
  PO_PAIR_LOOP(q, n) {
    PO_LOAD_BOUNDS(b, q, n);
    const double2 p = ld2(px, q, n), l = ld2(pzl, q, n), u = ld2(pzu, q, n);
    st2(cl, q, n, make_double2(e0.L ? p.x * l.x : 0.0, e1.L ? p.y * l.y : 0.0));
    st2(cu, q, n, make_double2(e0.U ? p.x * u.x : 0.0, e1.U ? p.y * u.y : 0.0));
  }
}
int k_corrector(Ctx *c, const Bounds &b, const double *px, const double *pzl, const double *pzu,
                int64_t n, double *cl, double *cu) {
  count_bytes(c, 8 - uniform_bound_streams(b), n);
  if (n <= 0) return PO_OK;
  PO_LAUNCH(corrector_kernel, grid_for(c, n), b, px, pzl, pzu, n, cl, cu);
  return PO_OK;
}

template <int NVB>
__global__ void __launch_bounds__(kBlock)
    corr_d1_dots_kernel(Bounds b, const double *__restrict__ px, const double *__restrict__ pzl,
                        const double *__restrict__ pzu, const double *__restrict__ rx,
                        const double *__restrict__ dinv, double beta_mu, PtrTable V, int64_t n,
                        double *__restrict__ t, double *__restrict__ partials) {
  __shared__ double sm[4 * NVB];
  double acc[NVB];
  const double *vp[NVB];
#pragma unroll
  for (int j = 0; j < NVB; j++) {
    acc[j] = 0.0;
    vp[j] = V.p[j];
  }
  PO_PAIR_LOOP(q, n) {
    PO_LOAD_BOUNDS(b, q, n);
// ... 1693 lines not shown
```

paropt_amd/csrc/wgram.hip:

```cpp
#include "core.hpp"

#include <math.h>
#include <stdlib.h>

#include <memory>
#include <vector>

namespace po {

typedef double f64x2 __attribute__((ext_vector_type(2)));

constexpr int kGramTile = 128;
constexpr int kGramLd = kGramTile + 8;

struct PtrTableW {
  double *p[kMaxPanel];
};

__device__ __forceinline__ f64x2 ld_nt(const double *p) {
  return __builtin_nontemporal_load(reinterpret_cast<const f64x2 *>(p));
}

template <int NG>
struct GramPlan {
  int owner[NG];
  int load[4];
  constexpr GramPlan() : owner{}, load{0, 0, 0, 0} {
    for (int J = NG - 1; J >= 0; J--) {
      int best = 0;
      for (int w = 1; w < 4; w++)
        if (load[w] < load[best]) best = w;
      owner[J] = best;
      load[best] += J + 1;
    }
  }
  constexpr int max_load() const {
    int m = load[0];
    for (int w = 1; w < 4; w++)
      if (load[w] > m) m = load[w];
    return m;
  }
};
template <int NG>
struct GramPlanHolder {
  static constexpr GramPlan<NG> plan = GramPlan<NG>();
  static constexpr int NQ = plan.max_load();
};

template <int NG, int LD = kGramLd>
__device__ __forceinline__ void gram_fetch(const double *__restrict__ base, const double *__restrict__ dwl, int s,
                                           double (&a)[NG], double &w) {
  w = dwl[16 * s];
#pragma unroll
  for (int g = 0; g < NG; g++) a[g] = base[(4 * g) * LD + 16 * s];
}

template <int NG, int W>
__device__ __forceinline__ void gram_step(const double (&a)[NG], double w, bool tsel,
                                          double (&acc)[GramPlanHolder<NG>::NQ]) {
  constexpr GramPlan<NG> plan = GramPlanHolder<NG>::plan;
  int q = 0;
#pragma unroll
  for (int J = 0; J < NG; J++) {
    if (plan.owner[J] == W) {
      const double bw = a[J] * ((J == NG - 1 && tsel) ? 1.0 : w);
#pragma unroll
      for (int I = 0; I <= J; I++) {
        acc[q] = __builtin_amdgcn_mfma_f64_4x4x4f64(a[I], bw, acc[q], 0, 0, 0);
        q++;
      }
    }
  }
}

template <int NG, int W, int TR = kGramTile, int LD = kGramLd>
__device__ __forceinline__ void gram_tile(const double *__restrict__ pt, const double *__restrict__ dw, int lane,
                                          int tcol, double (&acc)[GramPlanHolder<NG>::NQ]) {
  const int ci = lane & 3;
  const int rowoff = ((lane >> 2) & 3) + 4 * (lane >> 4);
  const double *base = pt + ci * LD + rowoff;
  const double *dwl = dw + rowoff;
  const bool tsel = (4 * (NG - 1) + ci == tcol);
  double a0[NG], a1[NG], w0, w1;
  gram_fetch<NG, LD>(base, dwl, 0, a0, w0);
#pragma unroll 1
  for (int s = 0; s < TR / 16; s += 2) {
    gram_fetch<NG, LD>(base, dwl, s + 1, a1, w1);
    gram_step<NG, W>(a0, w0, tsel, acc);
    if (s + 2 < TR / 16) gram_fetch<NG, LD>(base, dwl, s + 2, a0, w0);
    gram_step<NG, W>(a1, w1, tsel, acc);
  }
}

constexpr int kGramRowSplitMaxNG = 14;
constexpr int kGramRowSplitMinNG = 5;
constexpr int kGramPcMinNG = 6;
static_assert(kGramPcMinNG >= kGramRowSplitMinNG, "a producer/consumer panel narrower than the row split");

template <int NG>
__device__ __forceinline__ void gram_step_all(const double (&a)[NG], double w, bool tsel,
                                              double (&acc)[NG * (NG + 1) / 2]) {
  int q = 0;
#pragma unroll
  for (int J = 0; J < NG; J++) {
    const double bw = a[J] * ((J == NG - 1 && tsel) ? 1.0 : w);
#pragma unroll
    for (int I = 0; I <= J; I++) {
      acc[q] = __builtin_amdgcn_mfma_f64_4x4x4f64(a[I], bw, acc[q], 0, 0, 0);
      q++;
    }
  }
}

struct GramNoHook {
  __device__ __forceinline__ void operator()() const {}
};
template <int NG, class Hook = GramNoHook>
__device__ __forceinline__ void gram_tile_rows(const double *__restrict__ pt, const double *__restrict__ dw, int lane,
                                               int wave, int tcol, double (&acc)[NG * (NG + 1) / 2],
                                               const Hook &between = Hook()) {
  const int ci = lane & 3;
  const int rowoff = ((lane >> 2) & 3) + 4 * (lane >> 4);
  const double *base = pt + ci * kGramLd + rowoff;
  const double *dwl = dw + rowoff;
  const bool tsel = (4 * (NG - 1) + ci == tcol);
  double a0[NG], a1[NG], w0, w1;
  int off1 = 16 * (2 * wave + 1);
  asm volatile("" : "+v"(off1));
  if constexpr (NG <= 12) {
    gram_fetch<NG>(base, dwl, 2 * wave, a0, w0);
    gram_fetch<NG>(base + off1, dwl + off1, 0, a1, w1);
    between();
    gram_step_all<NG>(a0, w0, tsel, acc);
    gram_step_all<NG>(a1, w1, tsel, acc);
  } else {
    gram_fetch<NG>(base, dwl, 2 * wave, a0, w0);
    between();
    gram_step_all<NG>(a0, w0, tsel, acc);
    gram_fetch<NG>(base + off1, dwl + off1, 0, a0, w0);
    gram_step_all<NG>(a0, w0, tsel, acc);
  }
}

template <int NG>
__device__ __forceinline__ void gram_store_rows(const double (&acc)[NG * (NG + 1) / 2], int lane, int wave,
                                                double *__restrict__ red ) {
  constexpr int NP = NG * (NG + 1) / 2;
  int q = 0;
#pragma unroll
  for (int J = 0; J < NG; J++) {
#pragma unroll
    for (int I = 0; I <= J; I++) {
      const int p = I * NG - (I * (I - 1)) / 2 + (J - I);
      double v = acc[q];
      v += __shfl_xor(v, 4, 64);
      v += __shfl_xor(v, 8, 64);
      if (((lane >> 2) & 3) == 0) red[(size_t)wave * NP * 16 + p * 16 + (lane >> 4) * 4 + (lane & 3)] = v;
      q++;
    }
  }
}

template <int NG, int W>
__device__ __forceinline__ void gram_store(const double (&acc)[GramPlanHolder<NG>::NQ], int lane,
                                           double *__restrict__ partials) {
  constexpr GramPlan<NG> plan = GramPlanHolder<NG>::plan;
  int q = 0;
#pragma unroll
  for (int J = 0; J < NG; J++) {
    if (plan.owner[J] == W) {
#pragma unroll
      for (int I = 0; I <= J; I++) {
        const int p = I * NG - (I * (I - 1)) / 2 + (J - I);
        double v = acc[q];
        v += __shfl_xor(v, 4, 64);
        v += __shfl_xor(v, 8, 64);
        if (((lane >> 2) & 3) == 0) {
          const int slot = p * 16 + (lane >> 4) * 4 + (lane & 3);
          partials[(size_t)slot * gridDim.x + blockIdx.x] = v;
// ... 82 lines not shown
      case 2: gram_tile<NG, 2>(pt, dw, lane, tcol, acc); break;
      default: gram_tile<NG, 3>(pt, dw, lane, tcol, acc); break;
    }
  }
#undef PO_GRAM_PREFETCH
  switch (wave) {
    case 0: gram_store<NG, 0>(acc, lane, partials); break;
    case 1: gram_store<NG, 1>(acc, lane, partials); break;
    case 2: gram_store<NG, 2>(acc, lane, partials); break;
    default: gram_store<NG, 3>(acc, lane, partials); break;
  }
}

constexpr int kGramDepth = 3;
#ifdef PO_WGRAM_NO_FULL_STAGE
#define PO_WGRAM_FULL_STAGE 0
#else
#define PO_WGRAM_FULL_STAGE 1
#endif

__device__ unsigned long long g_wgram_stamp[8];

struct GramGeom {
  int64_t ngt = 0;
  int64_t rg = 0;
  int64_t nwcon = 0;
  int trows = kGramTile, G = 0, period = 0, nw = 0, ncols = 0;
  double alpha = 0.0;
};
__device__ __forceinline__ void gram_tile_geom(const GramGeom &gg, int64_t tile, int64_t &row0, int &nrows) {
  const bool grp = tile < gg.ngt;
  const int64_t rowg = tile * gg.trows, rowp = gg.rg + (tile - gg.ngt) * kGramTile;
  const int64_t left = gg.rg - rowg;
  const int nrg = left < gg.trows ? (int)left : gg.trows;
  row0 = grp ? rowg : rowp;
  nrows = grp ? nrg : kGramTile;
}
constexpr int kGramGroupNw = 24;
struct GramGroupOps {
  double p[kGramGroupNw], w[kGramGroupNw];
};
__device__ __forceinline__ void gram_groups_request(const double *__restrict__ pt, const double *__restrict__ dw,
                                                    const GramGeom &gg, int u, int gi, GramGroupOps &o) {
  const double *row = pt + u * kGramLd + gi * gg.period;
  const double *wr = dw + gi * gg.period;
#pragma unroll
  for (int k = 0; k < kGramGroupNw; k++) {
    if (k < gg.nw) {
      o.p[k] = row[k];
      o.w[k] = wr[k];
    }
  }
}
__device__ __forceinline__ double gram_groups_sum(const GramGeom &gg, const GramGroupOps &o) {
#pragma clang fp contract(off)
  double sacc = 0.0;
#pragma unroll
  for (int k = 0; k < kGramGroupNw; k++) {
    if (k < gg.nw) {
      const double prod = o.w[k] * o.p[k];
      sacc = sacc + prod;
    }
  }
  return gg.alpha * sacc;
}
__device__ __forceinline__ void gram_groups_rest(const double *__restrict__ pt, const double *__restrict__ dw,
                                                 const GramGeom &gg, double *const *Utab, int64_t g0, int ng, int ctid) {
#pragma clang fp contract(off)
  typedef __attribute__((address_space(1))) double gdouble;
  for (int pair = ctid + 256; pair < ng * gg.ncols; pair += 256) {
    const int u = pair / ng, gi = pair - u * ng;
    const double *row = pt + u * kGramLd + gi * gg.period;
    const double *wr = dw + gi * gg.period;
    double sacc = 0.0;
    for (int k = 0; k < gg.nw; k++) {
      const double prod = wr[k] * row[k];
      sacc = sacc + prod;
    }
    gdouble *up = (gdouble *)Utab[u];
    up[g0 + gi] = gg.alpha * sacc;
  }
}

template <int NG, int ZP>
struct GramProducer {
  f64x2 buf[kGramDepth][NG];
  f64x2 sbuf[kGramDepth][ZP > 0 ? ZP : 1];
  f64x2 dbuf[kGramDepth];
  int64_t row[kGramDepth];
  bool in[kGramDepth];
};

template <int NG, int ZP, int R>
__device__ __forceinline__ void gram_pc_load(GramProducer<NG, ZP> &P, const double *const (&colp)[NG],
                                             const double *const (&scol)[ZP > 0 ? ZP : 1], const double *d,
                                             int64_t tile, int64_t ntiles, int64_t n, int64_t ilast, int lane,
                                             const GramGeom &gg) {
  if (tile >= ntiles) {
    P.in[R] = false;
    return;
  }
  int64_t row0;
  int nrows;
  gram_tile_geom(gg, tile, row0, nrows);
  int64_t i = row0 + 2 * lane;
  const bool in = (2 * lane < nrows) && (i < n);
  int64_t alt = row0 + 2 * (lane & 3);
  alt = alt > ilast ? ilast : alt;
  if (!in) i = gg.ngt > 0 ? alt : ilast;
  P.in[R] = in;
  P.row[R] = i;
#pragma unroll
  for (int it = 0; it < NG; it++) P.buf[R][it] = ld_nt(colp[it] + i);
  if (ZP > 0) {
#pragma unroll
    for (int it = 0; it < ZP; it++) P.sbuf[R][it] = ld_nt(scol[it] + i);
  }
  P.dbuf[R] = *reinterpret_cast<const f64x2 *>(d + i);
}

template <int NG, int ZP, int R, bool FULL = false>
__device__ __forceinline__ void gram_pc_stage(GramProducer<NG, ZP> &P, double *__restrict__ pt,
                                              double *__restrict__ dw, double *const (&zcol)[ZP > 0 ? ZP : 1], int pw,
                                              int nv, int kpend, double b0, int lane) {
  const bool in = FULL ? true : P.in[R];
#pragma unroll
  for (int it = 0; it < NG; it++) {
    const int j = pw + 4 * it;
    f64x2 v = P.buf[R][it];
    if (ZP > 0 && it < ZP && j < kpend) {
      v.x -= b0 * P.sbuf[R][it].x;
      v.y -= b0 * P.sbuf[R][it].y;
      if (in && zcol[it]) __builtin_nontemporal_store(v, reinterpret_cast<f64x2 *>(zcol[it] + P.row[R]));
    }
    if (!FULL && !in) v = (f64x2){0.0, 0.0};
    if (j < nv) *reinterpret_cast<f64x2 *>(pt + j * kGramLd + 2 * lane) = v;
  }
  if (pw == 0) *reinterpret_cast<f64x2 *>(dw + 2 * lane) = in ? P.dbuf[R] : (f64x2){0.0, 0.0};
}

template <int NG, int ZP, int RS, int GS>
__global__ void __launch_bounds__(512, 1)
    wgram_pc_kernel(const double *__restrict__ d, PtrTable V, int nv, int64_t n, int64_t ntiles,
                    double *__restrict__ partials, PtrTable S, PtrTableW Zout, int kpend, double b0, int tcol,
                    int ablate, int prio, GramGeom gg, PtrTableW Ugs) {
  constexpr int M = 4 * NG;
  constexpr int NQ = GramPlanHolder<NG>::NQ;
  const bool want_stamps = (ablate & 16) != 0;
  ablate &= 15;
  if constexpr (GS == 0) gg = GramGeom();
  constexpr int kBufDoubles = M * kGramLd + kGramTile;
  extern __shared__ double lds[];
  const int tid = threadIdx.x, lane = tid & 63;
  const int wave = __builtin_amdgcn_readfirstlane(tid >> 6);
  for (int b2 = 0; b2 < 2; b2++)
    for (int idx = tid; idx < (M - nv) * kGramLd; idx += 512) lds[b2 * kBufDoubles + nv * kGramLd + idx] = 0.0;
  double **utab = reinterpret_cast<double **>(lds + 2 * kBufDoubles);
  if constexpr (GS != 0) {
    if (tid < kMaxPanel) utab[tid] = Ugs.p[tid];
  }
  int64_t first = blockIdx.x, stride = gridDim.x;
  int64_t nt = first < ntiles ? (ntiles - first + stride - 1) / stride : 0;
  if constexpr (GS != 0) {
    const int64_t per = (ntiles + gridDim.x - 1) / gridDim.x;
    first = blockIdx.x * per;
    stride = 1;
    nt = ntiles - first;
    nt = nt < 0 ? 0 : (nt < per ? nt : per);
  }
  __syncthreads();
  if (wave >= 4) {
    if (prio == 1) __builtin_amdgcn_s_setprio(1);
    if (prio == 2) __builtin_amdgcn_s_setprio(2);
    if (prio == 3) __builtin_amdgcn_s_setprio(3);
    const int pw = wave - 4;
    const double *colp[NG];
#pragma unroll
    for (int it = 0; it < NG; it++) {
      const int j = pw + 4 * it;
      colp[it] = V.p[j < nv ? j : nv - 1];
    }
    const double *scol[ZP > 0 ? ZP : 1];
    double *zcol[ZP > 0 ? ZP : 1];
#pragma unroll
    for (int it = 0; it < (ZP > 0 ? ZP : 1); it++) {
      const int j = pw + 4 * it;
      scol[it] = (ZP > 0 && kpend > 0) ? S.p[j < kpend ? j : kpend - 1] : nullptr;
      zcol[it] = (ZP > 0 && j < kpend) ? Zout.p[j] : nullptr;
    }
    const int64_t ilast = ((n - 1) >> 1) << 1;
    GramProducer<NG, ZP> P;
    gram_pc_load<NG, ZP, 0>(P, colp, scol, d, first, ntiles, n, ilast, lane, gg);
    gram_pc_load<NG, ZP, 1>(P, colp, scol, d, first + stride, ntiles, n, ilast, lane, gg);
    gram_pc_load<NG, ZP, 2>(P, colp, scol, d, first + 2 * stride, ntiles, n, ilast, lane, gg);
    unsigned long long st_stage = 0, st_load = 0, st_wait = 0;
    const bool stamp = want_stamps && blockIdx.x == 0 && wave == 4;
    const unsigned long long st_c0 = stamp ? __builtin_amdgcn_s_memtime() : 0;
    const unsigned long long st_r0 = stamp ? __builtin_amdgcn_s_memrealtime() : 0;
#define PO_PC_STEP(R)                                                                                         \
  if (it + (R) < nt) {                                                                                        \
    double *bt = lds + (size_t)((it + (R)) & 1) * kBufDoubles;                                                \
    const unsigned long long _t0 = stamp ? __builtin_amdgcn_s_memtime() : 0;                                  \
    if (ablate == 2) {                                                                                        \
      if (P.buf[R][0].x == 1.2345e301) bt[0] = P.buf[R][NG - 1].y;                                            \
    } else if (PO_WGRAM_FULL_STAGE && __all(P.in[R])) {                                                       \
      gram_pc_stage<NG, ZP, (R), true>(P, bt, bt + M * kGramLd, zcol, pw, nv, kpend, b0, lane);               \
    } else {                                                                                                  \
      gram_pc_stage<NG, ZP, (R), false>(P, bt, bt + M * kGramLd, zcol, pw, nv, kpend, b0, lane);              \
    }                                                                                                         \
    if (stamp) __builtin_amdgcn_s_waitcnt(0);                                                                 \
    const unsigned long long _t1 = stamp ? __builtin_amdgcn_s_memtime() : 0;                                  \
    if (ablate != 3) gram_pc_load<NG, ZP, (R)>(P, colp, scol, d, first + (it + (R) + kGramDepth) * stride, ntiles, n, ilast, lane, gg); \
    const unsigned long long _t2 = stamp ? __builtin_amdgcn_s_memtime() : 0;                                  \
    __syncthreads();                                                                                          \
    if (stamp) {                                                                                              \
      const unsigned long long _t3 = __builtin_amdgcn_s_memtime();                                            \
      st_stage += _t1 - _t0;                                                                                  \
      st_load += _t2 - _t1;                                                                                   \
      st_wait += _t3 - _t2;                                                                                   \
    }                                                                                                         \
  }
    for (int64_t it = 0; it < nt; it += kGramDepth) {
      PO_PC_STEP(0)
      PO_PC_STEP(1)
      PO_PC_STEP(2)
    }
#undef PO_PC_STEP
    if (stamp && lane == 0) {
      g_wgram_stamp[2] = st_stage;
      g_wgram_stamp[3] = st_load;
      g_wgram_stamp[4] = st_wait;
      g_wgram_stamp[5] = (unsigned long long)nt;
      g_wgram_stamp[6] = __builtin_amdgcn_s_memtime() - st_c0;
      g_wgram_stamp[7] = __builtin_amdgcn_s_memrealtime() - st_r0;
    }
    __syncthreads();
    if (RS) __syncthreads();
  } else {
    constexpr int NACC = RS ? NG * (NG + 1) / 2 : NQ;
    double acc[NACC];
#pragma unroll
    for (int q = 0; q < NACC; q++) acc[q] = 0.0;
    unsigned long long sc_wait = 0, sc_work = 0;
    const bool cstamp = want_stamps && blockIdx.x == 0 && wave == 0;
    [[maybe_unused]] int gs_u = 0, gs_gi = 0;
    if constexpr (GS == 1) {
      gs_u = tid / gg.G;
      gs_gi = tid - gs_u * gg.G;
    }
    for (int64_t it = 0; it < nt; it++) {
      const unsigned long long _t0 = cstamp ? __builtin_amdgcn_s_memtime() : 0;
      __syncthreads();
      const unsigned long long _t1 = cstamp ? __builtin_amdgcn_s_memtime() : 0;
      const double *bt = lds + (size_t)(it & 1) * kBufDoubles;
      if (ablate == 1) continue;
      [[maybe_unused]] GramGroupOps gops;
      [[maybe_unused]] bool gs_on = false, gs_mine = false;
      [[maybe_unused]] int gs_ng = 0, pu = 0, pgi = 0;
      [[maybe_unused]] int64_t gs_g0 = 0;
      if constexpr (GS == 1) {
        const int64_t tile = first + it * stride;
        gs_on = tile < gg.ngt;
        if (gs_on) {
          gs_g0 = tile * gg.G;
          gs_ng = (int)((gg.nwcon - gs_g0) < gg.G ? (gg.nwcon - gs_g0) : gg.G);
          pu = gs_u;
          pgi = gs_gi;
          if (gs_ng != gg.G) {
            pu = tid / gs_ng;
            pgi = tid - pu * gs_ng;
          }
          gs_mine = tid < gs_ng * gg.ncols;
          if (!RS && gs_mine && ablate != 5) gram_groups_request(bt, bt + M * kGramLd, gg, pu, pgi, gops);
        }
      }
      if constexpr (RS) {
        if constexpr (GS == 1) {
          auto request = [&]() {
            if (gs_on && gs_mine && ablate != 5) gram_groups_request(bt, bt + M * kGramLd, gg, pu, pgi, gops);
          };
          gram_tile_rows<NG>(bt, bt + M * kGramLd, lane, wave, tcol, acc, request);
        } else {
          gram_tile_rows<NG>(bt, bt + M * kGramLd, lane, wave, tcol, acc);
        }
      } else {
        switch (wave) {
          case 0: gram_tile<NG, 0>(bt, bt + M * kGramLd, lane, tcol, acc); break;
          case 1: gram_tile<NG, 1>(bt, bt + M * kGramLd, lane, tcol, acc); break;
          case 2: gram_tile<NG, 2>(bt, bt + M * kGramLd, lane, tcol, acc); break;
          default: gram_tile<NG, 3>(bt, bt + M * kGramLd, lane, tcol, acc); break;
        }
      }
      if constexpr (GS == 1) {
        if (gs_on) {
          if (gs_mine && ablate != 6) {
// ... 130 lines not shown
    } else {                                                                             \
      _Pragma("unroll") for (int h = 0; h < NH; h++) {                                   \
        f64x2 v = P.buf[R][h];                                                           \
        if (!_in) v = (f64x2){0.0, 0.0};                                                 \
        const int _j = j0 + 8 * h;                                                       \
        if (_j < nv) *reinterpret_cast<f64x2 *>(bt + _j * kG64Ld + 2 * rp) = v;          \
      }                                                                                  \
    }                                                                                    \
    if (pw == 0 && half == 0)                                                            \
      *reinterpret_cast<f64x2 *>(bt + M * kG64Ld + 2 * rp) = _in ? P.dbuf[R] : (f64x2){0.0, 0.0}; \
    if (stamp) __builtin_amdgcn_s_waitcnt(0xc07f);  \
    const unsigned long long _t1 = stamp ? __builtin_amdgcn_s_memtime() : 0;             \
    PO_G64_LOAD(R, first + (it + (R) + D) * stride);                                     \
    const unsigned long long _t2 = stamp ? __builtin_amdgcn_s_memtime() : 0;             \
    __syncthreads();                                                                     \
    if (stamp) {                                                                         \
      const unsigned long long _t3 = __builtin_amdgcn_s_memtime();                       \
      st_stage += _t1 - _t0;                                                             \
      st_load += _t2 - _t1;                                                              \
      st_wait += _t3 - _t2;                                                              \
    }                                                                                    \
  }
    PO_G64_LOAD(0, first);
    PO_G64_LOAD(1, first + stride);
    PO_G64_LOAD(2, first + 2 * stride);
    if constexpr (D == 4) PO_G64_LOAD(3, first + 3 * stride);
    int64_t it = 0;
    for (; it + D <= nt; it += D) {
      PO_G64_STEP(0)
      PO_G64_STEP(1)
      PO_G64_STEP(2)
      if constexpr (D == 4) PO_G64_STEP(3)
    }
    if (it < nt) PO_G64_STEP(0)
    if (it + 1 < nt) PO_G64_STEP(1)
    if constexpr (D == 4) {
      if (it + 2 < nt) PO_G64_STEP(2)
    }
#undef PO_G64_STEP
#undef PO_G64_LOAD
    if (stamp && lane == 0) {
      g_wgram_stamp[2] = st_stage;
      g_wgram_stamp[3] = st_load;
      g_wgram_stamp[4] = st_wait;
      g_wgram_stamp[5] = (unsigned long long)nt;
      g_wgram_stamp[6] = __builtin_amdgcn_s_memtime() - st_c0;
      g_wgram_stamp[7] = __builtin_amdgcn_s_memrealtime() - st_r0;
    }
    __syncthreads();
  } else {
    switch (wave) {
      case 0: gram64_consume<NG, 0>(lds, nt, partials, tcol, lane, want_stamps && blockIdx.x == 0); break;
      case 1: gram64_consume<NG, 1>(lds, nt, partials, tcol, lane, false); break;
      case 2: gram64_consume<NG, 2>(lds, nt, partials, tcol, lane, false); break;
      default: gram64_consume<NG, 3>(lds, nt, partials, tcol, lane, false); break;
    }
  }
}

template <int NG>
static int wgram_pc64_launch_t(Ctx *c, const double *d, const PtrTable &pt, int nv, int64_t n, int tcol, int ablate,
                               int prio, int *grid_out) {
  const size_t lds = (size_t)2 * (4 * NG * kG64Ld + kG64Tile) * sizeof(double);
  static bool attr_set = false;
  if (!attr_set) {
    PO_HIP(hipFuncSetAttribute(reinterpret_cast<const void *>(wgram_pc64_kernel<NG>),
                               hipFuncAttributeMaxDynamicSharedMemorySize, (int)lds));
    attr_set = true;
  }
  const int64_t ntiles = (n + kG64Tile - 1) / kG64Tile;
  int64_t g = (int64_t)c->num_cu;
  if (g > ntiles) g = ntiles;
  if (g < 1) g = 1;
  PO_TRY(ensure_partials(c, (size_t)g * (NG * (NG + 1) / 2) * 16));
  const int stamps = (ablate & 16) != 0;
  hipLaunchKernelGGL((wgram_pc64_kernel<NG>), dim3((int)g), dim3(512), lds, c->stream, d, pt, nv, n, ntiles,
                     c->d_partials, tcol, prio, stamps);
  c->n_launches++;
  PO_HIP(hipGetLastError());
  *grid_out = (int)g;
  return PO_OK;
}

template <int NG, int ZP, int RS, int GS = 0>
static int wgram_pc_launch_t(Ctx *c, const double *d, const PtrTable &pt, int nv, int64_t n, int64_t ntiles,
                             const PtrTable &st, const PtrTableW &zt, int kpend, double b0, int tcol, int ablate,
                             int prio, int *grid_out, const GramGeom *gg = nullptr, const PtrTableW *ut = nullptr) {
  const size_t lds = (size_t)2 * (4 * NG * kGramLd + kGramTile) * sizeof(double) + (GS ? kMaxPanel * sizeof(double *) : 0);
  static bool attr_set = false;
  if (!attr_set) {
    PO_HIP(hipFuncSetAttribute(reinterpret_cast<const void *>(wgram_pc_kernel<NG, ZP, RS, GS>),
                               hipFuncAttributeMaxDynamicSharedMemorySize, (int)lds));
    attr_set = true;
  }
  int64_t g = (int64_t)c->num_cu;
  if (g > ntiles) g = ntiles;
  if (g < 1) g = 1;
  PO_TRY(ensure_partials(c, (size_t)g * (NG * (NG + 1) / 2) * 16));
  static const PtrTableW no_u = PtrTableW();
  hipLaunchKernelGGL((wgram_pc_kernel<NG, ZP, RS, GS>), dim3((int)g), dim3(512), lds, c->stream, d, pt, nv, n, ntiles,
                     c->d_partials, st, zt, kpend, b0, tcol, ablate, prio, gg ? *gg : GramGeom(), ut ? *ut : no_u);
  c->n_launches++;
  PO_HIP(hipGetLastError());
  *grid_out = (int)g;
  return PO_OK;
}

template <int NG, int ZP, int OCC>
static int wgram_launch_t(Ctx *c, const double *d, const PtrTable &pt, int nv, int64_t n, int64_t ntiles,
                          const PtrTable &st, const PtrTableW &zt, int kpend, double b0, int tcol, int ablate,
                          int *grid_out) {
  const size_t lds = (size_t)(4 * NG * kGramLd + kGramTile) * sizeof(double);
  static bool attr_set = false;
  if (!attr_set) {
    PO_HIP(hipFuncSetAttribute(reinterpret_cast<const void *>(wgram_kernel<NG, ZP, OCC>),
                               hipFuncAttributeMaxDynamicSharedMemorySize, (int)lds));
    attr_set = true;
  }
  int per_cu = (int)((160 * 1024) / lds);
  if (per_cu > OCC) per_cu = OCC;
  if (per_cu < 1) per_cu = 1;
  int64_t g = (int64_t)c->num_cu * per_cu;
  if (g > ntiles) g = ntiles;
  if (g < 1) g = 1;
  PO_TRY(ensure_partials(c, (size_t)g * (NG * (NG + 1) / 2) * 16));
  hipLaunchKernelGGL((wgram_kernel<NG, ZP, OCC>), dim3((int)g), dim3(kBlock), lds, c->stream, d, pt, nv, n, ntiles,
                     c->d_partials, st, zt, kpend, b0, tcol, ablate);
  c->n_launches++;
  PO_HIP(hipGetLastError());
  *grid_out = (int)g;
  return PO_OK;
}

static int wgram_groups(int nv) { return (nv + 3) / 4; }

static bool wgram_groups_geom(const GramGroups *g, int nv, int64_t n, int kpend, GramGeom *gg) {
  if (!g || g->nwcon <= 0 || g->ncols <= 0 || g->ncols > nv || !g->U || kpend > 0) return false;
  const int64_t period = (int64_t)g->nw + g->skip;
  if (g->start != 0 || g->nw <= 0 || g->nw > kGramGroupNw || period > kGramTile) return false;
  if ((g->nwcon - 1) * period + g->nw > n) return false;
  int G = (int)(kGramTile / period);
  if (period & 1) G &= ~1;
  if (G < 1) return false;
  int64_t rg = g->nwcon * period;
  if (rg > n) rg = n;
  if ((rg & 1) && rg != n) return false;
  const int NG = (nv + 3) / 4;
  if (NG > 9 || n < 4 * kGramTile) return false;
  gg->ngt = (g->nwcon + G - 1) / G;
  gg->rg = rg;
  gg->nwcon = g->nwcon;
  gg->trows = G * (int)period;
  gg->G = G;
  gg->period = (int)period;
  gg->nw = g->nw;
  gg->ncols = g->ncols;
  gg->alpha = g->alpha;
  return true;
}

int k_wgram_launch(Ctx *c, const double *d, const double *const *V, int nv, int64_t n, int *nblocks,
                   int *nslots, const double *const *S, double *const *Zout, int kpend, double b0,
                   int preweighted_last, const GramGroups *groups, bool *groups_done) {
  if (groups_done) *groups_done = false;
  if (nv > kWgramMaxVecs || nv < 1) {
    set_error("wgram panel width %d outside 1..%d", nv, kWgramMaxVecs);
    return PO_ERR_ARG;
  }
  if (kpend > 12 || kpend > nv || (kpend > 0 && (!S || !Zout))) {
    set_error("wgram: %d pending columns cannot be materialised in the Gram pass", kpend);
    return PO_ERR_ARG;
  }
  count_bytes(c, nv + 1 + 2 * kpend, n);
  const int tcol = preweighted_last ? nv - 1 : -1;
  const int NG = wgram_groups(nv);
  int64_t ntiles = (n + kGramTile - 1) / kGramTile;
  PtrTable pt, st;
  PtrTableW zt, ut;
  for (int j = 0; j < kMaxPanel; j++) {
    pt.p[j] = j < nv ? V[j] : nullptr;
    st.p[j] = (S && j < kpend) ? S[j] : nullptr;
    zt.p[j] = (Zout && j < kpend) ? Zout[j] : nullptr;
    ut.p[j] = nullptr;
  }
  int grid = 0;
  GramGeom gg;
  const int ablate = dbg_switch(SW_WGRAM_ABLATE), prio = dbg_switch(SW_WGRAM_PRIO);
  if (NG >= kGramPcMinNG && wgram_groups_geom(groups, nv, n, kpend, &gg)) {
    ntiles = gg.ngt + (n - gg.rg + kGramTile - 1) / kGramTile;
    for (int j = 0; j < gg.ncols; j++) ut.p[j] = groups->U[j];
    count_bytes(c, (double)gg.ncols, gg.nwcon);
#define PO_WGG(NGv)                                                                                              \
  case NGv:                                                                                                      \
    PO_TRY((wgram_pc_launch_t<NGv, 0, 1, 1>(c, d, pt, nv, n, ntiles, st, zt, 0, 0.0, tcol, ablate, prio, &grid, &gg, \
                                            &ut)));                                                              \
    break;
    switch (NG) {
      PO_WGG(6) PO_WGG(7) PO_WGG(8) PO_WGG(9)
    }
#undef PO_WGG
    if (groups_done) *groups_done = true;
    *nblocks = grid;
    *nslots = (NG * (NG + 1) / 2) * 16;
    return PO_OK;
  }
#define PO_WG(NGv)                                                                                     \
  case NGv: {                                                                                          \
                         \
            \
    constexpr int OCC0 = NGv <= 8 ? 4 : (NGv <= 10 ? 3 : (NGv <= 14 ? 2 : 1));                         \
    constexpr int OCCZ = NGv <= 7 ? 3 : (NGv <= 13 ? 2 : 1);                                           \
            \
    constexpr int NGc = NGv < kGramPcMinNG ? kGramPcMinNG : (NGv <= 16 ? NGv : 16);                    \
    constexpr int NGr = NGc <= kGramRowSplitMaxNG ? NGc : kGramRowSplitMaxNG;                          \
    constexpr int NGo = NGc > kGramRowSplitMaxNG ? NGc : kGramRowSplitMaxNG + 1;                       \
    if (NGv >= 17 && kpend == 0 && n >= 4 * kGramTile) {                                               \
      constexpr int NGw = NGv >= 17 ? NGv : 17;                                                        \
      PO_TRY((wgram_pc64_launch_t<NGw>(c, d, pt, nv, n, tcol, ablate, prio, &grid)));                  \
    } else if (NGv <= 16 && NGv >= kGramPcMinNG && n >= 4 * kGramTile) {                               \
      if (NGv <= kGramRowSplitMaxNG) {                                                                 \
        if (kpend > 0) PO_TRY((wgram_pc_launch_t<NGr, 3, 1>(c, d, pt, nv, n, ntiles, st, zt, kpend, b0, tcol, ablate, prio, &grid))); \
        else PO_TRY((wgram_pc_launch_t<NGr, 0, 1>(c, d, pt, nv, n, ntiles, st, zt, 0, 0.0, tcol, ablate, prio, &grid)));              \
      } else if (kpend > 0 && NGv == 16)  \
        PO_TRY((wgram_launch_t<NGv, 3, 1>(c, d, pt, nv, n, ntiles, st, zt, kpend, b0, tcol, ablate, &grid)));                   \
      else if (kpend > 0) PO_TRY((wgram_pc_launch_t<(NGo < 16 ? NGo : 15), 3, 0>(c, d, pt, nv, n, ntiles, st, zt, kpend, b0, tcol, ablate, prio, &grid))); \
      else PO_TRY((wgram_pc_launch_t<NGo, 0, 0>(c, d, pt, nv, n, ntiles, st, zt, 0, 0.0, tcol, ablate, prio, &grid)));                \
    } else if (kpend > 0) {                                                                            \
      PO_TRY((wgram_launch_t<NGv, 3, OCCZ>(c, d, pt, nv, n, ntiles, st, zt, kpend, b0, tcol, ablate, &grid))); \
    } else {                                                                                           \
      PO_TRY((wgram_launch_t<NGv, 0, OCC0>(c, d, pt, nv, n, ntiles, st, zt, 0, 0.0, tcol, ablate, &grid)));    \
    }                                                                                                  \
  } break;
  switch (NG) {
    PO_WG(1) PO_WG(2) PO_WG(3) PO_WG(4) PO_WG(5) PO_WG(6) PO_WG(7) PO_WG(8) PO_WG(9) PO_WG(10)
    PO_WG(11) PO_WG(12) PO_WG(13) PO_WG(14) PO_WG(15) PO_WG(16) PO_WG(17) PO_WG(18) PO_WG(19) PO_WG(20)
  }
#undef PO_WG
  *nblocks = grid;
  *nslots = (NG * (NG + 1) / 2) * 16;
  return PO_OK;
}

int wgram_debug_stamps(double out[8]) {
  unsigned long long h[8] = {0, 0, 0, 0, 0, 0, 0, 0};
  PO_HIP(hipMemcpyFromSymbol(h, HIP_SYMBOL(g_wgram_stamp), sizeof(h)));
  for (int i = 0; i < 8; i++) out[i] = (double)h[i];
  return PO_OK;
}

static int wgram_one_launch(Ctx *c, const double *d, const double *const *V, int nv, int64_t n, double *W,
                            const double *const *S, double *const *Zout, int kpend, double b0, int preweighted_last,
                            bool may_defer, const GramGroups *groups = nullptr, bool *groups_done = nullptr);

int k_wgram(Ctx *c, const double *d, const double *const *V, int nv, int64_t n, double *W,
            const double *const *S, double *const *Zout, int kpend, double b0, int preweighted_last, bool may_defer,
            const GramGroups *groups, bool *groups_done) {
  if (groups_done) *groups_done = false;
  if (nv <= 0) return PO_OK;
  if (nv <= kWgramMaxVecs)
    return wgram_one_launch(c, d, V, nv, n, W, S, Zout, kpend, b0, preweighted_last, may_defer, groups, groups_done);
  if (kpend > 0 || preweighted_last) {
    set_error("wgram: a panel of %d columns is processed in blocks, which cannot form L-SR1 columns or carry a "
              "pre-weighted column", nv);
    return PO_ERR_ARG;
  }
  const int half = kWgramMaxVecs / 2;
  const int nb = (nv + half - 1) / half;
  int bw = (nv + nb - 1) / nb;
  bw = ((bw + 3) / 4) * 4;
  std::vector<const double *> V2;
  std::vector<double> W2;
  for (int I = 0; I < nb; I++) {
    const int i0 = I * bw, ni = (nv - i0 < bw) ? nv - i0 : bw;
    if (ni <= 0) continue;
    for (int J = I + 1; J < nb; J++) {
      const int j0 = J * bw, nj = (nv - j0 < bw) ? nv - j0 : bw;
      if (nj <= 0) continue;
      const int m2 = ni + nj;
      V2.assign(V + i0, V + i0 + ni);
      V2.insert(V2.end(), V + j0, V + j0 + nj);
      W2.assign((size_t)m2 * m2, 0.0);
      PO_TRY(wgram_one_launch(c, d, V2.data(), m2, n, W2.data(), nullptr, nullptr, 0, 0.0, 0, false));
      auto col = [&](int q) { return q < ni ? i0 + q : j0 + (q - ni); };
      for (int q = 0; q < m2; q++)
        for (int r = 0; r < m2; r++) W[col(r) + (size_t)nv * col(q)] = W2[r + (size_t)m2 * q];
    }
  }
  return PO_OK;
}

static int wgram_one_launch(Ctx *c, const double *d, const double *const *V, int nv, int64_t n, double *W,
                            const double *const *S, double *const *Zout, int kpend, double b0, int preweighted_last,
                            bool may_defer, const GramGroups *groups, bool *groups_done) {
  if (nv <= 0) return PO_OK;
  int grid = 0, nslots = 0;
  const bool defer = may_defer && c->batch_depth > 0;
  const bool timed = c->time_wgram != 0 && !defer;
  if (timed) PO_HIP(hipEventRecord(c->ev0, c->stream));
  PO_TRY(k_wgram_launch(c, d, V, nv, n, &grid, &nslots, S, Zout, kpend, b0, preweighted_last, groups, groups_done));
  if (timed) PO_HIP(hipEventRecord(c->ev1, c->stream));
  auto blocks = std::make_shared<std::vector<double>>(nslots);
  PO_TRY(reduce_finish(c, grid, nslots, 0, 0, blocks->data(), !defer));
  if (timed) {
    float ms = 0.0f;
    PO_HIP(hipEventSynchronize(c->ev1));
    PO_HIP(hipEventElapsedTime(&ms, c->ev0, c->ev1));
    const int w = kpend > 0 ? 1 : 0;
    c->wgram_ms[w] += ms;
    c->wgram_count[w]++;
    c->wgram_cols[w] = nv;
    c->wgram_bytes[w] += 8.0 * (double)n * (nv + 1 + 2 * kpend);
  }
  auto unpack = [blocks, nv, W] {
    const int NG = wgram_groups(nv);
    int p = 0;
    for (int I = 0; I < NG; I++) {
      for (int J = I; J < NG; J++, p++) {
        for (int i = 0; i < 4; i++) {
          for (int j = 0; j < 4; j++) {
            const int r = 4 * I + i, s = 4 * J + j;
            if (r < nv && s < nv && r <= s) {
              const double v = (*blocks)[(size_t)p * 16 + i * 4 + j];
              W[r + (size_t)nv * s] = v;
              W[s + (size_t)nv * r] = v;
            }
          }
        }
      }
    }
  };
  after_reduce(c, unpack);
  return PO_OK;
}

constexpr int kXgramMaxVecs = 48;

template <int NG, int W>
struct XgramOwn {
  static constexpr int NJ = W < NG ? (NG - W + 3) / 4 : 0;
  static constexpr int NQ = NJ * NG > 0 ? NJ * NG : 1;
};

template <int NG, int NJ>
__device__ __forceinline__ void xgram_fetch(const double *__restrict__ ub, const double *__restrict__ zb, int off,
                                            double (&a)[NG], double (&b)[NJ]) {
#pragma unroll
  for (int g = 0; g < NG; g++) a[g] = ub[(4 * g) * kG64Ld + off];
#pragma unroll
  for (int jj = 0; jj < NJ; jj++) b[jj] = zb[(16 * jj) * kG64Ld + off];
}
template <int NG, int NJ>
__device__ __forceinline__ void xgram_step(const double (&a)[NG], const double (&b)[NJ],
                                           double (&acc)[XgramOwn<NG, 0>::NQ]) {
  int q = 0;
#pragma unroll
  for (int jj = 0; jj < NJ; jj++) {
#pragma unroll
    for (int I = 0; I < NG; I++) {
      acc[q] = __builtin_amdgcn_mfma_f64_4x4x4f64(a[I], b[jj], acc[q], 0, 0, 0);
      q++;
    }
  }
}

template <int NG, int W>
__device__ __forceinline__ void xgram_tile(const double *__restrict__ ut, const double *__restrict__ zt, int lane,
                                           double (&acc)[XgramOwn<NG, 0>::NQ]) {
  constexpr int NJ = XgramOwn<NG, W>::NJ;
  if constexpr (NJ > 0) {
    const int ci = lane & 3;
    const int rowoff = ((lane >> 2) & 3) + 4 * (lane >> 4);
    const double *ub = ut + ci * kG64Ld + rowoff;
    const double *zb = zt + (4 * W + ci) * kG64Ld + rowoff;
    int off1 = 16;
    asm volatile("" : "+v"(off1));
    double a[NG], b[NJ];
#pragma unroll 1
    for (int s = 0; s < kG64Tile / 16; s += 2) {
      xgram_fetch<NG, NJ>(ub, zb, 16 * s, a, b);
      xgram_step<NG, NJ>(a, b, acc);
      xgram_fetch<NG, NJ>(ub, zb, 16 * s + off1, a, b);
      xgram_step<NG, NJ>(a, b, acc);
    }
  }
}

template <int NG, int W>
__device__ __forceinline__ void xgram_store(const double (&acc)[XgramOwn<NG, 0>::NQ], int lane,
                                            double *__restrict__ partials) {
  constexpr int NJ = XgramOwn<NG, W>::NJ;
  int q = 0;
#pragma unroll
  for (int jj = 0; jj < NJ; jj++) {
#pragma unroll
    for (int I = 0; I < NG; I++) {
      const int p = I * NG + (W + 4 * jj);
      double v = acc[q];
      v += __shfl_xor(v, 4, 64);
      v += __shfl_xor(v, 8, 64);
      if (((lane >> 2) & 3) == 0) {
        const int slot = p * 16 + (lane >> 4) * 4 + (lane & 3);
        partials[(size_t)slot * gridDim.x + blockIdx.x] = v;
      }
      q++;
    }
  }
}

template <int NG, int OCC>
__global__ void __launch_bounds__(kBlock, OCC)
    xgram_kernel(PtrTable U, PtrTable Z, int nvu, int nvz, int64_t n, int64_t ntiles,
                 double *__restrict__ partials) {
  constexpr int M = 4 * NG;
  extern __shared__ double lds[];
  const int tid = threadIdx.x, lane = tid & 63;
// ... 136 lines not shown
```

Before: 44.73.

## Fold Dinv and t formation into the weighted Gram pass for large n

When the problem exceeds the Infinity Cache size, the separate dinv/d1 kernel that writes Dinv and t is deferred. Instead, the producer/consumer Gram kernel computes Dinv and t on the fly from x, bounds, multipliers and rx, which removes one full write-then-reread pass over the vectors. Later consumers call ensureDinvT to materialise the vectors lazily when they actually need them. This adds bookkeeping state, a restricted set of eligible panel shapes, and the risk of recomputing Dinv/t twice when a later step needs them stored.

```diff
diff --git a/paropt_amd/csrc/bound_elem.hpp b/paropt_amd/csrc/bound_elem.hpp
--- /dev/null
+++ b/paropt_amd/csrc/bound_elem.hpp
@@ -0,0 +1,36 @@
+#pragma once
+
+namespace po {
+
+struct BE {
+  bool L, U;
+  double xl, xu, zl, zu;
+};
+__device__ __forceinline__ BE bound_elem(double x, double lb, double ub, double zl, double zu,
+                                         double maxb, int use_lower, int use_upper) {
+  BE e;
+  e.L = use_lower && (lb > -maxb);
+  e.U = use_upper && (ub < maxb);
+  e.xl = e.L ? (x - lb) : 1.0;
+  e.xu = e.U ? (ub - x) : 1.0;
+  e.zl = zl;
+  e.zu = zu;
+  return e;
+}
+
+__device__ __forceinline__ double dinv_elem(const BE &e, double diag) {
+  double v = diag;
+  if (e.L) v += e.zl / e.xl;
+  if (e.U) v += e.zu / e.xu;
+  return 1.0 / v;
+}
+
+__device__ __forceinline__ double d1_elem(const BE &e, double rx, double beta_mu, double cl = 0.0,
+                                          double cu = 0.0) {
+  double d1 = rx;
+  if (e.L) d1 += (-(e.xl * e.zl - beta_mu) - cl) / e.xl;
+  if (e.U) d1 -= (-(e.xu * e.zu - beta_mu) + cu) / e.xu;
+  return d1;
+}
+
+}
diff --git a/paropt_amd/csrc/capi.cpp b/paropt_amd/csrc/capi.cpp
--- a/paropt_amd/csrc/capi.cpp
+++ b/paropt_amd/csrc/capi.cpp
@@ -82,6 +82,42 @@
   return PO_OK;
 }
 int po_debug_wgram_stamps(double *out8) { return po::wgram_debug_stamps(out8); }
+int po_debug_wgram_fold(int folded, po_vec d, const po_vec *vecs, int nvecs, const po_vec *S, const po_vec *Zout,
+                        int kpend, double b0, po_vec x, po_vec lb, po_vec ub, po_vec zl, po_vec zu, po_vec rx,
+                        int use_lower, int use_upper, int lb_uni, double lb_c, int ub_uni, double ub_c,
+                        double max_bound, double diag, double beta_mu, double *W) {
+  PO_CHECK_PTR(d);
+  PO_CHECK_PTR(vecs);
+  PO_CHECK_PTR(W);
+  const po_vec bound_vecs[6] = {x, lb, ub, zl, zu, rx};
+  for (po_vec v : bound_vecs) {
+    PO_CHECK_PTR(v);
+    if (v->n != d->n || v->ctx != d->ctx) return PO_ERR_ARG;
+  }
+  if (nvecs < 2 || nvecs > po::kMaxPanel || kpend < 0 || kpend > nvecs - 1 || (kpend > 0 && (!S || !Zout))) return PO_ERR_ARG;
+  std::vector<const double *> p(nvecs), s(kpend > 0 ? kpend : 1);
+  std::vector<double *> z(kpend > 0 ? kpend : 1);
+  for (int j = 0; j < nvecs; j++) {
+    PO_CHECK_PTR(vecs[j]);
+    if (vecs[j]->n != d->n || vecs[j]->ctx != d->ctx) return PO_ERR_ARG;
+    p[j] = vecs[j]->d;
+  }
+  for (int j = 0; j < kpend; j++) {
+    PO_CHECK_PTR(S[j]);
+    PO_CHECK_PTR(Zout[j]);
+    if (S[j]->n != d->n || Zout[j]->n != d->n) return PO_ERR_ARG;
+    s[j] = S[j]->d;
+    z[j] = Zout[j]->d;
+  }
+  po::GramFold f;
+  f.b = po::Bounds{x->d, lb->d, ub->d, zl->d, zu->d, max_bound, use_lower, use_upper, lb_uni, ub_uni, lb_c, ub_c};
+  f.rx = rx->d;
+  f.diag = diag;
+  f.beta_mu = beta_mu;
+  if (!folded) PO_TRY(po::k_dinv_d1(d->ctx, f.b, diag, nullptr, rx->d, beta_mu, d->n, d->d, vecs[nvecs - 1]->d));
+  return po::k_wgram_pc_debug(d->ctx, d->d, p.data(), nvecs, d->n, W, kpend > 0 ? s.data() : nullptr,
+                              kpend > 0 ? z.data() : nullptr, kpend, b0, folded ? &f : nullptr);
+}
 int po_debug_set_switch(int id, int value) {
   po::dbg_switch_set(id, value);
   return PO_OK;
diff --git a/paropt_amd/csrc/context.cpp b/paropt_amd/csrc/context.cpp
--- a/paropt_amd/csrc/context.cpp
+++ b/paropt_amd/csrc/context.cpp
@@ -65,6 +65,7 @@
     {SW_SYNC_TRACE, "PAROPT_AMD_SYNC_TRACE", 0, true},
     {SW_USER_TIMING, "PAROPT_AMD_USER_TIMING", 0, true},
     {SW_DUMP_LONG_SOLVES, "PAROPT_AMD_DUMP_LONG_SOLVES", -1, false},
+    {SW_GRAM_FOLD, "PAROPT_AMD_GRAM_FOLD", -1, false},
 };
 static struct {
   int value = -1;
diff --git a/paropt_amd/csrc/core.hpp b/paropt_amd/csrc/core.hpp
--- a/paropt_amd/csrc/core.hpp
+++ b/paropt_amd/csrc/core.hpp
@@ -41,6 +41,7 @@
   unsigned long long serial = 0;
   hipStream_t stream = nullptr;
   int num_cu = 256;
+  static constexpr double kInfinityCacheBytes = 256.0 * 1024.0 * 1024.0;
   int max_blocks = 2048;
   int rank = 0, size = 1;
   CommKind comm_kind = COMM_SELF;
@@ -181,7 +182,7 @@
   SW_NO_FUSED_MERIT = 23, SW_NO_LEAN_STEP = 24, SW_NO_RECOMPUTE_DT = 25, SW_NO_FUSED_UPDATE = 26,
   SW_NO_CSR_GROUPS = 27, SW_NO_FRONTS = 28, SW_FORCE_RCCL = 29, SW_RCCL_ALLGATHER = 30, SW_NO_DIRECT_RED = 31,
   SW_NO_FLAG_POLL = 32, SW_NO_BATCH = 33, SW_HOST_TRACE = 34, SW_SYNC_TRACE = 35, SW_USER_TIMING = 36,
-  SW_DUMP_LONG_SOLVES = 37, SW_COUNT = 38
+  SW_DUMP_LONG_SOLVES = 37, SW_GRAM_FOLD = 38, SW_COUNT = 39
 };
 int dbg_switch(DbgSwitch id);
 void dbg_switch_set(int id, int value);
@@ -273,17 +274,22 @@
   int ncols = 0;
   double *const *U = nullptr;
 };
+struct GramFold;
+bool wgram_fold_form(int nv, int64_t n, int kpend, const GramGroups *groups);
 int k_wgram(Ctx *c, const double *d, const double *const *V, int nv, int64_t n, double *W,
             const double *const *S = nullptr, double *const *Zout = nullptr, int kpend = 0,
             double b0 = 0.0, int preweighted_last = 0, bool may_defer = false,
-            const GramGroups *groups = nullptr, bool *groups_done = nullptr);
+            const GramGroups *groups = nullptr, bool *groups_done = nullptr, const GramFold *fold = nullptr);
+int k_wgram_pc_debug(Ctx *c, const double *d, const double *const *V, int nv, int64_t n, double *W,
+                     const double *const *S, double *const *Zout, int kpend, double b0, const GramFold *fold);
 int wgram_debug_stamps(double out[8]);
 int k_xgram(Ctx *c, const double *const *U, const double *const *Z, int m, int64_t w, double *out,
             bool may_defer = false);
 int k_wgram_launch(Ctx *c, const double *d, const double *const *V, int nv, int64_t n,
                    int *nblocks, int *nslots, const double *const *S = nullptr,
                    double *const *Zout = nullptr, int kpend = 0, double b0 = 0.0,
-                   int preweighted_last = 0, const GramGroups *groups = nullptr, bool *groups_done = nullptr);
+                   int preweighted_last = 0, const GramGroups *groups = nullptr, bool *groups_done = nullptr,
+                   const GramFold *fold = nullptr, bool force_pc = false);
 
 struct Bounds {
   const double *x, *lb, *ub, *zl, *zu;
@@ -293,6 +299,11 @@
   double lb_c = 0.0, ub_c = 0.0;
 };
 inline int uniform_bound_streams(const Bounds &b) { return (b.lb_uni ? 1 : 0) + (b.ub_uni ? 1 : 0); }
+struct GramFold {
+  Bounds b;
+  const double *rx = nullptr;
+  double diag = 0.0, beta_mu = 0.0;
+};
 struct ResidualSums {
   double comp_prod = 0, comp_count = 0, l1_rx = 0, l1_rzl = 0, l1_rzu = 0, l2_rx = 0, l2_rzl = 0, l2_rzu = 0;
   double max_rx = 0, max_rzl = 0, max_rzu = 0;
diff --git a/paropt_amd/csrc/ip.cpp b/paropt_amd/csrc/ip.cpp
--- a/paropt_amd/csrc/ip.cpp
+++ b/paropt_amd/csrc/ip.cpp
@@ -612,9 +612,19 @@
   scratch_flags.spec_dt_valid = false;
   scratch_flags.t_is_plain_dinv_d1 = false;
   *formed = RHS_NONE;
+  fold_pending = false;
+  dinv_t_stored = true;
   if (want_t) {
     const bool left_behind = have_spec_dt && !use_hdiag && spec_dt_diag == diag && spec_dt_bmu == bmu;
-    if (!left_behind) PO_TRY(k_dinv_d1(ctx, bounds(), diag, h, rx->d, bmu, n, Dinv->d, tvec->d));
+    const int sw = dbg_switch(SW_GRAM_FOLD);
+    const bool past_cache = sw == 1 || (sw < 0 && 48.0 * (double)n > Ctx::kInfinityCacheBytes);
+    const bool solves_reform = forms.recompute_dt && forms.recompute_first_step && forms.recompute_rhs &&
+                               forms.analytic_panel_dots && options.integer("iterative_refinement_steps") > 0 &&
+                               !corrector_active && !inexact_newton_step;
+    fold_pending = !left_behind && !use_hdiag && past_cache && solves_reform;
+    fold_diag = diag;
+    fold_bmu = bmu;
+    if (!left_behind && !fold_pending) PO_TRY(k_dinv_d1(ctx, bounds(), diag, h, rx->d, bmu, n, Dinv->d, tvec->d));
     scratch_flags.t_is_plain_dinv_d1 = !use_hdiag;
     t0_diag = diag;
     *formed = RHS_T;
@@ -627,15 +637,24 @@
   return PO_OK;
 }
 
+int InteriorPoint::ensureDinvT() {
+  if (dinv_t_stored && !fold_pending) return PO_OK;
+  fold_pending = false;
+  dinv_t_stored = true;
+  return k_dinv_d1(ctx, bounds(), fold_diag, nullptr, rx->d, fold_bmu, n, Dinv->d, tvec->d);
+}
+
 int InteriorPoint::gramPass(const GramPlan &plan, bool *groups_done) {
   const int m = (int)plan.V.size(), mt = m + (plan.with_t ? 1 : 0), k = plan.kform;
   const bool with_t = plan.with_t;
   std::vector<const double *> V(plan.V);
   if (with_t) V.push_back(tvec->d);
   Wt_buf.assign((size_t)mt * mt, 0.0);
+  const GramFold fold{bounds(), rx->d, fold_diag, fold_bmu};
   PO_TRY(k_wgram(ctx, Dinv->d, V.data(), mt, n, Wt_buf.data(), k > 0 ? plan.S.data() : nullptr,
                  k > 0 ? plan.Zout.data() : nullptr, k, plan.b0, with_t ? 1 : 0, plan.may_defer, plan.groups,
-                 groups_done));
+                 groups_done, plan.fold ? &fold : nullptr));
+  if (plan.fold) dinv_t_stored = false;
   t0dots.assign(with_t ? m : 0, 0.0);
   after_reduce(ctx, [this, m, mt, k, with_t] {
     auto at = [&](int i) { return k == 0 ? i : (i < c ? k + i : i - c); };
@@ -698,6 +717,11 @@
   }
   plan.with_t = (fuse_t || fuse_tw) && m > 0 && m + 1 <= kWgramMaxVecs;
   plan.may_defer = wbatch.open;
+  if (fold_pending) {
+    plan.fold = plan.with_t && fuse_t && wgram_fold_form(m + 1, n, plan.kform, plan.groups);
+    if (plan.fold) fold_pending = false;
+    else PO_TRY(ensureDinvT());
+  }
   bool panel_done = false;
   kkt.W.assign((size_t)m * m, 0.0);
   t0dots.clear();
@@ -750,10 +774,14 @@
   std::vector<double> dots(m > 0 ? m : 1, 0.0);
   if (corr_fused) {
     need_panel();
+    PO_TRY(ensureDinvT());
     PO_TRY(k_corr_d1_dots(ctx, bounds(), px->d, pzl->d, pzu->d, rx->d, Dinv->d, beta_mu, P.data(), m, n, tvec->d,
                           dots.data()));
   } else {
-    if (!refine_pass && !have_t0) PO_TRY(k_d1(ctx, bounds(), rx->d, Dinv->d, beta_mu, n, tvec->d, cl, cu));
+    if (!refine_pass && !have_t0) {
+      PO_TRY(ensureDinvT());
+      PO_TRY(k_d1(ctx, bounds(), rx->d, Dinv->d, beta_mu, n, tvec->d, cl, cu));
+    }
     if (have_t0) {
       for (int i = 0; i < m; i++) dots[i] = t0dots[i];
     } else if (refine_pass && step_flags.tdots_valid && (int)tdots.size() == m) {
@@ -806,6 +834,7 @@
   const bool defer = forms.recompute_first_step;
   double *tp_out = !defer ? tvec->d : (forms.recompute_rhs ? nullptr : xt->d);
   const bool redo_dt1 = forms.recompute_dt && defer && forms.recompute_rhs && scratch_flags.first_t_recomputable;
+  if (!redo_dt1) PO_TRY(ensureDinvT());
   PO_TRY(k_solve2_dots(ctx, {.b = bounds(), .t = redo_dt1 ? nullptr : tvec->d, .dinv = Dinv->d,
                              .alpha = sp.alpha.data(), .coef2 = coef.data(), .P = sp.P.data(), .nv = m,
                              .beta_mu = sp.beta_mu, .tau = sp.tau, .rx = rx->d, .diag = diag, .n = n, .px = px->d,
@@ -828,6 +857,7 @@
   const bool take_merit = forms.fuse_merit && forms.recompute_rhs && !corr;
   const bool lean = forms.lean_step && lean_step_allowed && take_merit && iterate_flags.iterate_logs_valid;
   const bool redo_dt = forms.recompute_dt && forms.recompute_rhs && scratch_flags.first_t_recomputable;
+  if (!redo_dt) PO_TRY(ensureDinvT());
   if (lean) {
     step_flags.pz_stored = false;
     step_beta_mu = sp.beta_mu;
@@ -851,6 +881,7 @@
 
 int InteriorPoint::correctorSolve(const SolvePass &sp) {
   const bool want_logs = !iterate_flags.iterate_logs_valid;
+  PO_TRY(ensureDinvT());
   PO_TRY(k_solve2c(ctx, {.b = bounds(), .t = tvec->d, .dinv = Dinv->d, .alpha = sp.alpha.data(), .P = sp.P.data(),
                          .nv = sp.m, .beta_mu = sp.beta_mu, .tau = sp.tau, .n = n, .px = px->d, .pzl = pzl->d,
                          .pzu = pzu->d, .va = vA->d, .nca = c, .g = g->d, .want_logs = want_logs ? 1 : 0,
@@ -873,6 +904,7 @@
 
 int InteriorPoint::storedStepSolve(const SolvePass &sp, bool refine_pass, const double *coef2, double diag,
                                    const double *cl, const double *cu) {
+  PO_TRY(ensureDinvT());
   return k_solve2(ctx, {.b = bounds(), .t = tvec->d, .dinv = Dinv->d, .alpha = sp.alpha.data(), .P = sp.P.data(),
                         .nv = sp.m, .beta_mu = sp.beta_mu, .refine = refine_pass ? 1 : 0, .tau = sp.tau, .n = n,
                         .px = px->d, .pzl = pzl->d, .pzu = pzu->d, .out = step_mins, .coef2 = coef2, .rx = rx->d,
@@ -912,6 +944,7 @@
         Pq.get().push_back(tvec->d);
         coef[mres++] = 1.0;
       }
+      PO_TRY(ensureDinvT());
       PO_TRY(k_res_step(ctx, bounds(), rx->d, px->d, pzl->d, pzu->d, has_w ? nullptr : Dinv->d, coef.data(),
                         Pq.get().data(), mres, diag, beta_mu, n, has_w ? d1v->d : tvec->d));
     }
diff --git a/paropt_amd/csrc/ip.hpp b/paropt_amd/csrc/ip.hpp
--- a/paropt_amd/csrc/ip.hpp
+++ b/paropt_amd/csrc/ip.hpp
@@ -75,7 +75,7 @@
   const std::vector<double> &gramMatrix() const { return kkt.W; }
   const std::vector<int> &cPivots() const { return kkt.cpiv; }
   const double *stepMins() const { return step_mins; }
-  Vec *dinvVec() { return Dinv; }
+  Vec *dinvVec() { return ensureDinvT() == PO_OK ? Dinv : nullptr; }
   Vec *rxVec() { return rx; }
   void flushHistory();
   int checkGradients(double dh, std::string *report);
@@ -173,6 +173,9 @@
   double t0_mu = 0.0;
   std::vector<double> t0dots;
   double t0_diag = 0.0;
+  bool fold_pending = false, dinv_t_stored = true;
+  double fold_diag = 0.0, fold_bmu = 0.0;
+  int ensureDinvT();
 
   struct IterateFlags {
     bool ac_valid = false;
@@ -307,6 +310,7 @@
     std::vector<double *> Zout;
     double b0 = 0.0;
     bool with_t = false;
+    bool fold = false;
     const GramGroups *groups = nullptr;
     bool may_defer = false;
   };
diff --git a/paropt_amd/csrc/ip_gmres.cpp b/paropt_amd/csrc/ip_gmres.cpp
--- a/paropt_amd/csrc/ip_gmres.cpp
+++ b/paropt_amd/csrc/ip_gmres.cpp
@@ -19,6 +19,7 @@
   std::vector<const double *> P = panel(use_qn, &k);
   PO_TRY(kkt.checkWidth(k));
   const int m = c + k;
+  PO_TRY(ensureDinvT());
   PO_TRY(k_d1s(ctx, bounds(), bx, Dinv->d, alpha, beta_mu, n, tvec->d));
   std::vector<double> dots(m > 0 ? m : 1, 0.0);
   if (m > 0) PO_TRY(k_mdot(ctx, tvec->d, P.data(), m, n, dots.data()));
diff --git a/paropt_amd/csrc/kernels.hip b/paropt_amd/csrc/kernels.hip
--- a/paropt_amd/csrc/kernels.hip
+++ b/paropt_amd/csrc/kernels.hip
@@ -1,4 +1,6 @@
 #include "core.hpp"
+
+#include "bound_elem.hpp"
 
 #include <math.h>
 #include <stdlib.h>
@@ -788,21 +790,6 @@
 }
 
 
-struct BE {
-  bool L, U;
-  double xl, xu, zl, zu;
-};
-__device__ __forceinline__ BE bound_elem(double x, double lb, double ub, double zl, double zu,
-                                         double maxb, int use_lower, int use_upper) {
-  BE e;
-  e.L = use_lower && (lb > -maxb);
-  e.U = use_upper && (ub < maxb);
-  e.xl = e.L ? (x - lb) : 1.0;
-  e.xu = e.U ? (ub - x) : 1.0;
-  e.zl = zl;
-  e.zu = zu;
-  return e;
-}
 #define PO_MAKE_BOUNDS(b, q, n)                                                          \
   const bool _has2 = (2 * q + 1 < n);                                                    \
   const BE e0 = bound_elem(_x.x, _lb.x, _ub.x, _zl.x, _zu.x, (b).max_bound, (b).use_lower, \
@@ -951,12 +938,6 @@
   return reduce_finish(c, grid, 8, 0, 3, out);
 }
 
-__device__ __forceinline__ double dinv_elem(const BE &e, double diag) {
-  double v = diag;
-  if (e.L) v += e.zl / e.xl;
-  if (e.U) v += e.zu / e.xu;
-  return 1.0 / v;
-}
 __global__ void __launch_bounds__(kBlock)
     dinv_kernel(Bounds b, double diag, const double *__restrict__ hdiag, int64_t n,
                 double *__restrict__ dinv) {
@@ -974,13 +955,6 @@
   return PO_OK;
 }
 
-__device__ __forceinline__ double d1_elem(const BE &e, double rx, double beta_mu, double cl = 0.0,
-                                          double cu = 0.0) {
-  double d1 = rx;
-  if (e.L) d1 += (-(e.xl * e.zl - beta_mu) - cl) / e.xl;
-  if (e.U) d1 -= (-(e.xu * e.zu - beta_mu) + cu) / e.xu;
-  return d1;
-}
 __global__ void __launch_bounds__(kBlock)
     d1_kernel(Bounds b, const double *__restrict__ rx, const double *__restrict__ dinv,
               double beta_mu, const double *__restrict__ cl, const double *__restrict__ cu, int64_t n,
diff --git a/paropt_amd/csrc/wgram.hip b/paropt_amd/csrc/wgram.hip
--- a/paropt_amd/csrc/wgram.hip
+++ b/paropt_amd/csrc/wgram.hip
@@ -1,4 +1,6 @@
 #include "core.hpp"
+
+#include "bound_elem.hpp"
 
 #include <math.h>
 #include <stdlib.h>
@@ -95,6 +97,7 @@
 constexpr int kGramRowSplitMaxNG = 14;
 constexpr int kGramRowSplitMinNG = 5;
 constexpr int kGramPcMinNG = 6;
+constexpr int kGramFoldMaxNGZ = 12;
 static_assert(kGramPcMinNG >= kGramRowSplitMinNG, "a producer/consumer panel narrower than the row split");
 
 template <int NG>
@@ -343,20 +346,21 @@
   }
 }
 
-template <int NG, int ZP>
+template <int NG, int ZP, int FOLD = 0>
 struct GramProducer {
   f64x2 buf[kGramDepth][NG];
   f64x2 sbuf[kGramDepth][ZP > 0 ? ZP : 1];
   f64x2 dbuf[kGramDepth];
+  f64x2 fraw[FOLD ? 5 : 1];
   int64_t row[kGramDepth];
   bool in[kGramDepth];
 };
 
-template <int NG, int ZP, int R>
-__device__ __forceinline__ void gram_pc_load(GramProducer<NG, ZP> &P, const double *const (&colp)[NG],
+template <int NG, int ZP, int R, int FOLD = 0>
+__device__ __forceinline__ void gram_pc_load(GramProducer<NG, ZP, FOLD> &P, const double *const (&colp)[NG],
                                              const double *const (&scol)[ZP > 0 ? ZP : 1], const double *d,
                                              int64_t tile, int64_t ntiles, int64_t n, int64_t ilast, int lane,
-                                             const GramGeom &gg) {
+                                             const GramGeom &gg, const GramFold &fa, bool own) {
   if (tile >= ntiles) {
     P.in[R] = false;
     return;
@@ -377,13 +381,50 @@
 #pragma unroll
     for (int it = 0; it < ZP; it++) P.sbuf[R][it] = ld_nt(scol[it] + i);
   }
-  P.dbuf[R] = *reinterpret_cast<const f64x2 *>(d + i);
-}
-
-template <int NG, int ZP, int R, bool FULL = false>
-__device__ __forceinline__ void gram_pc_stage(GramProducer<NG, ZP> &P, double *__restrict__ pt,
+  if constexpr (!FOLD) {
+    P.dbuf[R] = *reinterpret_cast<const f64x2 *>(d + i);
+  } else if (own) {
+    P.fraw[0] = ld_nt(fa.b.x + i);
+    P.fraw[1] = ld_nt(fa.b.zl + i);
+    P.fraw[2] = ld_nt(fa.b.zu + i);
+    if (!fa.b.lb_uni) P.fraw[3] = ld_nt(fa.b.lb + i);
+    if (!fa.b.ub_uni) P.fraw[4] = ld_nt(fa.b.ub + i);
+  }
+}
+
+template <int NG, int ZP, int R>
+__device__ __forceinline__ void gram_fold_form(GramProducer<NG, ZP, 1> &P, const GramFold &fa, int64_t n) {
+  const Bounds &b = fa.b;
+  const f64x2 xv = P.fraw[0], zl = P.fraw[1], zu = P.fraw[2], r = P.buf[R][NG - 1];
+  const f64x2 lbv = b.lb_uni ? (f64x2){b.lb_c, b.lb_c} : P.fraw[3];
+  const f64x2 ubv = b.ub_uni ? (f64x2){b.ub_c, b.ub_c} : P.fraw[4];
+  const bool in = P.in[R], has2 = P.row[R] + 1 < n;
+  const BE e0 = bound_elem(xv.x, lbv.x, ubv.x, zl.x, zu.x, b.max_bound, b.use_lower, b.use_upper);
+  BE e1 = bound_elem(xv.y, lbv.y, ubv.y, zl.y, zu.y, b.max_bound, b.use_lower, b.use_upper);
+  if (!has2) {
+    e1.L = false;
+    e1.U = false;
+    e1.xl = 1.0;
+    e1.xu = 1.0;
+  }
+  f64x2 dv = (f64x2){dinv_elem(e0, fa.diag + 0.0), dinv_elem(e1, fa.diag + 0.0)};
+  f64x2 tv = (f64x2){dv.x * d1_elem(e0, r.x, fa.beta_mu), dv.y * d1_elem(e1, r.y, fa.beta_mu)};
+  if (!has2) {
+    dv.y = 0.0;
+    tv.y = 0.0;
+  }
+  if (!in) {
+    dv = (f64x2){0.0, 0.0};
+    tv = (f64x2){0.0, 0.0};
+  }
+  P.dbuf[R] = dv;
+  P.buf[R][NG - 1] = tv;
+}
+
+template <int NG, int ZP, int R, bool FULL = false, int FOLD = 0>
+__device__ __forceinline__ void gram_pc_stage(GramProducer<NG, ZP, FOLD> &P, double *__restrict__ pt,
                                               double *__restrict__ dw, double *const (&zcol)[ZP > 0 ? ZP : 1], int pw,
-                                              int nv, int kpend, double b0, int lane) {
+                                              int nv, int kpend, double b0, int lane, bool own) {
   const bool in = FULL ? true : P.in[R];
 #pragma unroll
   for (int it = 0; it < NG; it++) {
@@ -397,14 +438,19 @@
     if (!FULL && !in) v = (f64x2){0.0, 0.0};
     if (j < nv) *reinterpret_cast<f64x2 *>(pt + j * kGramLd + 2 * lane) = v;
   }
-  if (pw == 0) *reinterpret_cast<f64x2 *>(dw + 2 * lane) = in ? P.dbuf[R] : (f64x2){0.0, 0.0};
-}
-
-template <int NG, int ZP, int RS, int GS>
+  if constexpr (FOLD) {
+    if (own) *reinterpret_cast<f64x2 *>(dw + 2 * lane) = P.dbuf[R];
+  } else {
+    if (pw == 0) *reinterpret_cast<f64x2 *>(dw + 2 * lane) = in ? P.dbuf[R] : (f64x2){0.0, 0.0};
+  }
+}
+
+template <int NG, int ZP, int RS, int GS, int FOLD = 0>
 __global__ void __launch_bounds__(512, 1)
     wgram_pc_kernel(const double *__restrict__ d, PtrTable V, int nv, int64_t n, int64_t ntiles,
                     double *__restrict__ partials, PtrTable S, PtrTableW Zout, int kpend, double b0, int tcol,
-                    int ablate, int prio, GramGeom gg, PtrTableW Ugs) {
+                    int ablate, int prio, GramGeom gg, PtrTableW Ugs, GramFold fa) {
+  static_assert(!FOLD || (RS == 1 && GS == 0), "Dinv and t are formed in the row-split form without group sums only");
   constexpr int M = 4 * NG;
   constexpr int NQ = GramPlanHolder<NG>::NQ;
   const bool want_stamps = (ablate & 16) != 0;
@@ -435,6 +481,7 @@
     if (prio == 2) __builtin_amdgcn_s_setprio(2);
     if (prio == 3) __builtin_amdgcn_s_setprio(3);
     const int pw = wave - 4;
+    const bool own = FOLD && pw == (tcol & 3);
     const double *colp[NG];
 #pragma unroll
     for (int it = 0; it < NG; it++) {
@@ -450,10 +497,16 @@
       zcol[it] = (ZP > 0 && j < kpend) ? Zout.p[j] : nullptr;
     }
     const int64_t ilast = ((n - 1) >> 1) << 1;
-    GramProducer<NG, ZP> P;
-    gram_pc_load<NG, ZP, 0>(P, colp, scol, d, first, ntiles, n, ilast, lane, gg);
-    gram_pc_load<NG, ZP, 1>(P, colp, scol, d, first + stride, ntiles, n, ilast, lane, gg);
-    gram_pc_load<NG, ZP, 2>(P, colp, scol, d, first + 2 * stride, ntiles, n, ilast, lane, gg);
+    GramProducer<NG, ZP, FOLD> P;
+    gram_pc_load<NG, ZP, 0, FOLD>(P, colp, scol, d, first, ntiles, n, ilast, lane, gg, fa, own);
+    if constexpr (FOLD) {
+      if (own) gram_fold_form<NG, ZP, 0>(P, fa, n);
+    }
+    gram_pc_load<NG, ZP, 1, FOLD>(P, colp, scol, d, first + stride, ntiles, n, ilast, lane, gg, fa, own);
+    if constexpr (FOLD) {
+      if (own) gram_fold_form<NG, ZP, 1>(P, fa, n);
+    }
+    gram_pc_load<NG, ZP, 2, FOLD>(P, colp, scol, d, first + 2 * stride, ntiles, n, ilast, lane, gg, fa, own);
     unsigned long long st_stage = 0, st_load = 0, st_wait = 0;
     const bool stamp = want_stamps && blockIdx.x == 0 && wave == 4;
     const unsigned long long st_c0 = stamp ? __builtin_amdgcn_s_memtime() : 0;
@@ -465,13 +518,16 @@
     if (ablate == 2) {                                                                                        \
       if (P.buf[R][0].x == 1.2345e301) bt[0] = P.buf[R][NG - 1].y;                                            \
     } else if (PO_WGRAM_FULL_STAGE && __all(P.in[R])) {                                                       \
-      gram_pc_stage<NG, ZP, (R), true>(P, bt, bt + M * kGramLd, zcol, pw, nv, kpend, b0, lane);               \
+      gram_pc_stage<NG, ZP, (R), true, FOLD>(P, bt, bt + M * kGramLd, zcol, pw, nv, kpend, b0, lane, own);    \
     } else {                                                                                                  \
-      gram_pc_stage<NG, ZP, (R), false>(P, bt, bt + M * kGramLd, zcol, pw, nv, kpend, b0, lane);              \
+      gram_pc_stage<NG, ZP, (R), false, FOLD>(P, bt, bt + M * kGramLd, zcol, pw, nv, kpend, b0, lane, own);   \
+    }                                                                                                         \
+    if constexpr (FOLD) {  \
+      if (own) gram_fold_form<NG, ZP, ((R) + 2) % kGramDepth>(P, fa, n);                                      \
     }                                                                                                         \
     if (stamp) __builtin_amdgcn_s_waitcnt(0);                                                                 \
     const unsigned long long _t1 = stamp ? __builtin_amdgcn_s_memtime() : 0;                                  \
-    if (ablate != 3) gram_pc_load<NG, ZP, (R)>(P, colp, scol, d, first + (it + (R) + kGramDepth) * stride, ntiles, n, ilast, lane, gg); \
+    if (ablate != 3) gram_pc_load<NG, ZP, (R), FOLD>(P, colp, scol, d, first + (it + (R) + kGramDepth) * stride, ntiles, n, ilast, lane, gg, fa, own); \
     const unsigned long long _t2 = stamp ? __builtin_amdgcn_s_memtime() : 0;                                  \
     __syncthreads();                                                                                          \
     if (stamp) {                                                                                              \
@@ -768,14 +824,15 @@
   return PO_OK;
 }
 
-template <int NG, int ZP, int RS, int GS = 0>
+template <int NG, int ZP, int RS, int GS = 0, int FOLD = 0>
 static int wgram_pc_launch_t(Ctx *c, const double *d, const PtrTable &pt, int nv, int64_t n, int64_t ntiles,
                              const PtrTable &st, const PtrTableW &zt, int kpend, double b0, int tcol, int ablate,
-                             int prio, int *grid_out, const GramGeom *gg = nullptr, const PtrTableW *ut = nullptr) {
+                             int prio, int *grid_out, const GramGeom *gg = nullptr, const PtrTableW *ut = nullptr,
+                             const GramFold *fold = nullptr) {
   const size_t lds = (size_t)2 * (4 * NG * kGramLd + kGramTile) * sizeof(double) + (GS ? kMaxPanel * sizeof(double *) : 0);
   static bool attr_set = false;
   if (!attr_set) {
-    PO_HIP(hipFuncSetAttribute(reinterpret_cast<const void *>(wgram_pc_kernel<NG, ZP, RS, GS>),
+    PO_HIP(hipFuncSetAttribute(reinterpret_cast<const void *>(wgram_pc_kernel<NG, ZP, RS, GS, FOLD>),
                                hipFuncAttributeMaxDynamicSharedMemorySize, (int)lds));
     attr_set = true;
   }
@@ -784,8 +841,9 @@
   if (g < 1) g = 1;
   PO_TRY(ensure_partials(c, (size_t)g * (NG * (NG + 1) / 2) * 16));
   static const PtrTableW no_u = PtrTableW();
-  hipLaunchKernelGGL((wgram_pc_kernel<NG, ZP, RS, GS>), dim3((int)g), dim3(512), lds, c->stream, d, pt, nv, n, ntiles,
-                     c->d_partials, st, zt, kpend, b0, tcol, ablate, prio, gg ? *gg : GramGeom(), ut ? *ut : no_u);
+  hipLaunchKernelGGL((wgram_pc_kernel<NG, ZP, RS, GS, FOLD>), dim3((int)g), dim3(512), lds, c->stream, d, pt, nv, n,
+                     ntiles, c->d_partials, st, zt, kpend, b0, tcol, ablate, prio, gg ? *gg : GramGeom(),
+                     ut ? *ut : no_u, fold ? *fold : GramFold());
   c->n_launches++;
   PO_HIP(hipGetLastError());
   *grid_out = (int)g;
@@ -819,6 +877,10 @@
 }
 
 static int wgram_groups(int nv) { return (nv + 3) / 4; }
+
+static double wgram_streams(int nv, int kpend, const GramFold *fold) {
+  return fold ? nv - 1 + 2 * kpend + 6 - uniform_bound_streams(fold->b) : nv + 1 + 2 * kpend;
+}
 
 static bool wgram_groups_geom(const GramGroups *g, int nv, int64_t n, int kpend, GramGeom *gg) {
   if (!g || g->nwcon <= 0 || g->ncols <= 0 || g->ncols > nv || !g->U || kpend > 0) return false;
@@ -845,10 +907,30 @@
   return true;
 }
 
+bool wgram_fold_form(int nv, int64_t n, int kpend, const GramGroups *groups) {
+  const int NG = wgram_groups(nv);
+  GramGeom gg;
+  if (nv < 2 || nv > kWgramMaxVecs || kpend > 12 || kpend > nv - 1) return false;
+  if (NG < kGramPcMinNG || NG > kGramRowSplitMaxNG || n < 4 * kGramTile) return false;
+  if (kpend > 0 && NG > kGramFoldMaxNGZ) return false;
+  return !wgram_groups_geom(groups, nv, n, kpend, &gg);
+}
+
 int k_wgram_launch(Ctx *c, const double *d, const double *const *V, int nv, int64_t n, int *nblocks,
                    int *nslots, const double *const *S, double *const *Zout, int kpend, double b0,
-                   int preweighted_last, const GramGroups *groups, bool *groups_done) {
+                   int preweighted_last, const GramGroups *groups, bool *groups_done, const GramFold *fold,
+                   bool force_pc) {
   if (groups_done) *groups_done = false;
+  if (fold && !(preweighted_last && (force_pc || wgram_fold_form(nv, n, kpend, groups)))) {
+    set_error("wgram: this form of the pass (%d columns, n = %lld) does not form Dinv and t", nv, (long long)n);
+    return PO_ERR_ARG;
+  }
+  if (force_pc && (wgram_groups(nv) < kGramPcMinNG || wgram_groups(nv) > kGramRowSplitMaxNG || n < 1 ||
+                   (fold && kpend > 0 && wgram_groups(nv) > kGramFoldMaxNGZ))) {
+    set_error("wgram: the row-split producer/consumer form takes %d..%d columns, not %d", 4 * kGramPcMinNG - 3,
+              4 * kGramRowSplitMaxNG, nv);
+    return PO_ERR_ARG;
+  }
   if (nv > kWgramMaxVecs || nv < 1) {
     set_error("wgram panel width %d outside 1..%d", nv, kWgramMaxVecs);
     return PO_ERR_ARG;
@@ -857,7 +939,7 @@
     set_error("wgram: %d pending columns cannot be materialised in the Gram pass", kpend);
     return PO_ERR_ARG;
   }
-  count_bytes(c, nv + 1 + 2 * kpend, n);
+  count_bytes(c, wgram_streams(nv, kpend, fold), n);
   const int tcol = preweighted_last ? nv - 1 : -1;
   const int NG = wgram_groups(nv);
   int64_t ntiles = (n + kGramTile - 1) / kGramTile;
@@ -865,6 +947,7 @@
   PtrTableW zt, ut;
   for (int j = 0; j < kMaxPanel; j++) {
     pt.p[j] = j < nv ? V[j] : nullptr;
+    if (fold && j == nv - 1) pt.p[j] = fold->rx;
     st.p[j] = (S && j < kpend) ? S[j] : nullptr;
     zt.p[j] = (Zout && j < kpend) ? Zout[j] : nullptr;
     ut.p[j] = nullptr;
@@ -872,7 +955,7 @@
   int grid = 0;
   GramGeom gg;
   const int ablate = dbg_switch(SW_WGRAM_ABLATE), prio = dbg_switch(SW_WGRAM_PRIO);
-  if (NG >= kGramPcMinNG && wgram_groups_geom(groups, nv, n, kpend, &gg)) {
+  if (NG >= kGramPcMinNG && !force_pc && wgram_groups_geom(groups, nv, n, kpend, &gg)) {
     ntiles = gg.ngt + (n - gg.rg + kGramTile - 1) / kGramTile;
     for (int j = 0; j < gg.ncols; j++) ut.p[j] = groups->U[j];
     count_bytes(c, (double)gg.ncols, gg.nwcon);
@@ -903,9 +986,11 @@
     if (NGv >= 17 && kpend == 0 && n >= 4 * kGramTile) {                                               \
       constexpr int NGw = NGv >= 17 ? NGv : 17;                                                        \
       PO_TRY((wgram_pc64_launch_t<NGw>(c, d, pt, nv, n, tcol, ablate, prio, &grid)));                  \
-    } else if (NGv <= 16 && NGv >= kGramPcMinNG && n >= 4 * kGramTile) {                               \
+    } else if (NGv <= 16 && NGv >= kGramPcMinNG && (n >= 4 * kGramTile || force_pc)) {                 \
       if (NGv <= kGramRowSplitMaxNG) {                                                                 \
-        if (kpend > 0) PO_TRY((wgram_pc_launch_t<NGr, 3, 1>(c, d, pt, nv, n, ntiles, st, zt, kpend, b0, tcol, ablate, prio, &grid))); \
+        if (fold && kpend > 0) PO_TRY((wgram_pc_launch_t<(NGr <= kGramFoldMaxNGZ ? NGr : kGramFoldMaxNGZ), 3, 1, 0, 1>(c, d, pt, nv, n, ntiles, st, zt, kpend, b0, tcol, ablate, prio, &grid, nullptr, nullptr, fold))); \
+        else if (fold) PO_TRY((wgram_pc_launch_t<NGr, 0, 1, 0, 1>(c, d, pt, nv, n, ntiles, st, zt, 0, 0.0, tcol, ablate, prio, &grid, nullptr, nullptr, fold))); \
+        else if (kpend > 0) PO_TRY((wgram_pc_launch_t<NGr, 3, 1>(c, d, pt, nv, n, ntiles, st, zt, kpend, b0, tcol, ablate, prio, &grid))); \
         else PO_TRY((wgram_pc_launch_t<NGr, 0, 1>(c, d, pt, nv, n, ntiles, st, zt, 0, 0.0, tcol, ablate, prio, &grid)));              \
       } else if (kpend > 0 && NGv == 16)  \
         PO_TRY((wgram_launch_t<NGv, 3, 1>(c, d, pt, nv, n, ntiles, st, zt, kpend, b0, tcol, ablate, &grid)));                   \
@@ -936,15 +1021,17 @@
 
 static int wgram_one_launch(Ctx *c, const double *d, const double *const *V, int nv, int64_t n, double *W,
                             const double *const *S, double *const *Zout, int kpend, double b0, int preweighted_last,
-                            bool may_defer, const GramGroups *groups = nullptr, bool *groups_done = nullptr);
+                            bool may_defer, const GramGroups *groups = nullptr, bool *groups_done = nullptr,
+                            const GramFold *fold = nullptr, bool force_pc = false);
 
 int k_wgram(Ctx *c, const double *d, const double *const *V, int nv, int64_t n, double *W,
             const double *const *S, double *const *Zout, int kpend, double b0, int preweighted_last, bool may_defer,
-            const GramGroups *groups, bool *groups_done) {
+            const GramGroups *groups, bool *groups_done, const GramFold *fold) {
   if (groups_done) *groups_done = false;
   if (nv <= 0) return PO_OK;
   if (nv <= kWgramMaxVecs)
-    return wgram_one_launch(c, d, V, nv, n, W, S, Zout, kpend, b0, preweighted_last, may_defer, groups, groups_done);
+    return wgram_one_launch(c, d, V, nv, n, W, S, Zout, kpend, b0, preweighted_last, may_defer, groups, groups_done,
+                            fold);
   if (kpend > 0 || preweighted_last) {
     set_error("wgram: a panel of %d columns is processed in blocks, which cannot form L-SR1 columns or carry a "
               "pre-weighted column", nv);
@@ -977,13 +1064,15 @@
 
 static int wgram_one_launch(Ctx *c, const double *d, const double *const *V, int nv, int64_t n, double *W,
                             const double *const *S, double *const *Zout, int kpend, double b0, int preweighted_last,
-                            bool may_defer, const GramGroups *groups, bool *groups_done) {
+                            bool may_defer, const GramGroups *groups, bool *groups_done, const GramFold *fold,
+                            bool force_pc) {
   if (nv <= 0) return PO_OK;
   int grid = 0, nslots = 0;
   const bool defer = may_defer && c->batch_depth > 0;
   const bool timed = c->time_wgram != 0 && !defer;
   if (timed) PO_HIP(hipEventRecord(c->ev0, c->stream));
-  PO_TRY(k_wgram_launch(c, d, V, nv, n, &grid, &nslots, S, Zout, kpend, b0, preweighted_last, groups, groups_done));
+  PO_TRY(k_wgram_launch(c, d, V, nv, n, &grid, &nslots, S, Zout, kpend, b0, preweighted_last, groups, groups_done, fold,
+                        force_pc));
   if (timed) PO_HIP(hipEventRecord(c->ev1, c->stream));
   auto blocks = std::make_shared<std::vector<double>>(nslots);
   PO_TRY(reduce_finish(c, grid, nslots, 0, 0, blocks->data(), !defer));
@@ -995,7 +1084,7 @@
     c->wgram_ms[w] += ms;
     c->wgram_count[w]++;
     c->wgram_cols[w] = nv;
-    c->wgram_bytes[w] += 8.0 * (double)n * (nv + 1 + 2 * kpend);
+    c->wgram_bytes[w] += 8.0 * (double)n * wgram_streams(nv, kpend, fold);
   }
   auto unpack = [blocks, nv, W] {
     const int NG = wgram_groups(nv);
@@ -1017,6 +1106,15 @@
   };
   after_reduce(c, unpack);
   return PO_OK;
+}
+
+int k_wgram_pc_debug(Ctx *c, const double *d, const double *const *V, int nv, int64_t n, double *W,
+                     const double *const *S, double *const *Zout, int kpend, double b0, const GramFold *fold) {
+  if (nv < 2 || n < 1) {
+    set_error("wgram debug pass: %d columns, n = %lld", nv, (long long)n);
+    return PO_ERR_ARG;
+  }
+  return wgram_one_launch(c, d, V, nv, n, W, S, Zout, kpend, b0, 1, false, nullptr, nullptr, fold, true);
 }
 
 constexpr int kXgramMaxVecs = 48;
```

After: 45.28 (median of 6 runs). 1.01x the previous value.
